# linnil1/KIR_graph

Measured on AMD Instinct MI355X. Metric: typed 150 bp PE reads/s (pileup+EM) per GPU; achieved HBM GB/s vs roofline, higher is better.
Workload: dtype f64

## Files before the change

include/graphkir_hip.h:

```cpp
#ifndef GRAPHKIR_HIP_H
#define GRAPHKIR_HIP_H

#include <stddef.h>
#include <stdint.h>

#ifdef __cplusplus
extern "C" {
#endif

#define GK_ABI_VERSION 1

#define GK_OK 0
#define GK_ERR_NO_DEVICE (-1)
#define GK_ERR_HIP (-2)
#define GK_ERR_ARG (-3)
#define GK_ERR_ASSERT (-4)
#define GK_ERR_CAPACITY (-5)

#define GK_MAX_CIG 14
#define GK_MAX_MM 16
#define GK_MAX_INS 6
#define GK_MAX_EVENTS 22
#define GK_CIG_M 0
#define GK_CIG_I 1
// ... 47 lines not shown
typedef struct gk_tab gk_tab;
typedef struct gk_lut gk_lut;
typedef uint64_t gk_dptr;

int gk_abi_version(void);
const char* gk_last_error(void);
int gk_device_count(int* n);
int gk_ctx_create(int device, gk_ctx** out);
int gk_ctx_create_priority(int device, int urgent, gk_ctx** out);
int gk_ctx_destroy(gk_ctx* ctx);
int gk_sync(gk_ctx* ctx);
int gk_device_memory(gk_ctx* ctx, int64_t* free_bytes, int64_t* total_bytes, int64_t* pool_cached_bytes);
int gk_malloc(gk_ctx* ctx, size_t bytes, gk_dptr* out);
int gk_free(gk_ctx* ctx, gk_dptr p);
int gk_memset(gk_ctx* ctx, gk_dptr p, int value, size_t bytes);
int gk_h2d(gk_ctx* ctx, gk_dptr dst, const void* src, size_t bytes);
int gk_d2h(gk_ctx* ctx, void* dst, gk_dptr src, size_t bytes);
int gk_d2d(gk_ctx* ctx, gk_dptr dst, gk_dptr src, size_t bytes);
int gk_timer_start(gk_ctx* ctx);
int gk_timer_stop_ms(gk_ctx* ctx, float* ms);
int gk_prof_enable(gk_ctx* ctx, int on);
int gk_prof_kernel_count(void);
const char* gk_prof_kernel_name(int id);
int gk_prof_collect(gk_ctx* ctx, int64_t* launches, double* total_ms);

int gk_index_create(gk_ctx* ctx, const uint64_t* key, int32_t n_var, const int32_t* gene_vbeg,
                    int32_t n_gene, gk_index** out);
int gk_index_destroy(gk_index* idx);

typedef struct gk_tab_info {
  int64_t n_pairs;
  int64_t n_valid;
  int64_t n_ids;
  int32_t n_novel;
  int32_t err_flags;
  gk_dptr d_pair_src;
  gk_dptr d_off;
  gk_dptr d_ids;
  gk_dptr d_pair_gene;
  gk_dptr d_pair_nh;
  gk_dptr d_novel_key;
} gk_tab_info;
int gk_tabulate(gk_ctx* ctx, gk_index* idx, gk_dptr d_mates, int64_t n_pairs, gk_tab** out);
int gk_tabulate_corrected(gk_ctx* ctx, gk_index* idx, gk_dptr d_mates, int64_t n_pairs, gk_dptr d_corr,
                          gk_dptr d_gene_pos0, gk_tab** out);
int gk_tabulate_spilled(gk_ctx* ctx, gk_index* idx, gk_dptr d_mates, int64_t n_pairs, gk_dptr d_corr,
                        gk_dptr d_gene_pos0, const gk_mate_wide* wide, const int64_t* spill_pair, int64_t n_spill,
                        gk_tab** out);
#define GK_COMPACT_STAGE_WORDS 4352
int gk_tabulate_compact(gk_ctx* ctx, gk_index* idx, gk_dptr d_compact, int64_t n_pairs, gk_dptr d_corr,
                        gk_dptr d_gene_pos0, const gk_mate_wide* wide, const int64_t* spill_pair, int64_t n_spill,
                        gk_tab** out);
int gk_tab_from_csr(gk_ctx* ctx, int32_t n_var_total, int64_t n_valid, const uint32_t* off, const uint32_t* ids,
                    const uint8_t* pair_gene, const uint8_t* pair_nh, gk_tab** out);
int gk_tab_get_info(gk_tab* tab, gk_tab_info* info);
int gk_tab_destroy(gk_tab* tab);

int gk_select_gene(gk_ctx* ctx, gk_tab* tab, int gene, int multiple, gk_dptr d_rows_out, int64_t* n_out);
int gk_select_nonempty(gk_ctx* ctx, gk_tab* tab, gk_dptr d_rows, int64_t n_rows, gk_dptr d_vflag,
                       gk_dptr d_rows_out, int64_t* n_out);

int gk_variant_count(gk_ctx* ctx, gk_tab* tab, gk_dptr d_rows, int64_t n_rows, gk_dptr d_vflag,
                     gk_dptr d_cnt);
int gk_variant_count_range(gk_ctx* ctx, gk_tab* tab, gk_dptr d_rows, int64_t n_rows, gk_dptr d_vflag,
                           gk_dptr d_cnt, int32_t vbeg, int32_t vend);
int gk_variant_correct(gk_ctx* ctx, gk_tab* tab, gk_dptr d_cnt, gk_dptr d_vflag);
int gk_variant_surviving(gk_ctx* ctx, gk_tab* tab, gk_dptr d_cnt, gk_dptr d_vflag, int64_t max_out,
                         int32_t* ord_out, uint32_t* pos_out, uint32_t* neg_out, int64_t* n_out);

int gk_variant_surviving_gene(gk_ctx* ctx, gk_tab* tab, gk_dptr d_cnt, gk_dptr d_vflag, int32_t gene, int32_t vbeg,
                              int32_t vend, int64_t max_out, int32_t* ord_out, uint32_t* pos_out, uint32_t* neg_out,
                              int64_t* n_out);
int gk_sample_prepare(gk_ctx* ctx, gk_tab* tab, int32_t multiple, gk_dptr d_vflag, gk_dptr d_cnt, gk_dptr d_rows,
                      int64_t* gene_off_out);
int gk_sample_prepare_all(gk_ctx* ctx, gk_tab* tab, int32_t multiple, gk_dptr d_vflag, gk_dptr d_cnt, gk_dptr d_rows,
                          int64_t* gene_off_out, int64_t max_out, int32_t* ord_out, uint32_t* pos_out, uint32_t* neg_out,
                          int64_t* n_out, uint64_t* novel_key_out);
int gk_sample_prepare_exon(gk_ctx* ctx, gk_tab* tab, int32_t multiple, gk_dptr d_vflag, gk_dptr d_cnt, gk_dptr d_rows,
                           int64_t* gene_off_out, int64_t max_out, int32_t* ord_out, uint32_t* pos_out, uint32_t* neg_out,
                           int64_t* n_out);
int gk_sample_prepare_exon_from(gk_ctx* ctx, gk_tab* tab, int32_t multiple, gk_dptr d_vflag, gk_dptr d_cnt, gk_dptr d_rows,
                                int64_t* gene_off_out, int64_t max_out, int32_t* ord_out, uint32_t* pos_out,
                                uint32_t* neg_out, int64_t* n_out, gk_dptr d_cnt_full);

int gk_compat(gk_ctx* ctx, gk_tab* tab, gk_dptr d_rows, int64_t n_rows, gk_dptr d_vflag,
              int32_t vbeg, int32_t vend, gk_dptr d_mask, int32_t words, int32_t n_allele, int32_t keep_empty,
              gk_dptr d_probs, gk_dptr d_miss, gk_dptr d_nvar);

int gk_novel_assign(gk_ctx* ctx, gk_dptr d_probs, int64_t n_rows, int32_t n_cols, const uint32_t* col_entries,
                    int32_t n_entries, gk_dptr d_code, uint16_t* code_out, uint32_t* count_out, int32_t* first_out);
int gk_novel_confusion(gk_ctx* ctx, gk_tab* tab, gk_dptr d_rows, int64_t n_rows, gk_dptr d_code, gk_dptr d_vflag,
                       int32_t vbeg, int32_t vend, gk_dptr d_carry, const int32_t* entry_col, const int32_t* entry_slot,
                       int32_t n_entries, int32_t n_slots, uint64_t* totals_out, int64_t max_out, int32_t* slot_out,
                       int32_t* ord_out, uint32_t* count_out, uint64_t* key_out, int64_t* n_out);

int gk_lut_create(gk_ctx* ctx, int32_t log2_capacity, gk_lut** out);
int gk_lut_destroy(gk_lut* lut);
int gk_lut_collect(gk_lut* lut, gk_dptr d_vals, int64_t n);
int gk_lut_pending(gk_lut* lut, int32_t* n_total, int32_t* n_known);
int gk_lut_export(gk_lut* lut, int32_t first, int32_t count, double* keys_out);
int gk_lut_define(gk_lut* lut, int32_t first, int32_t count, const double* log_vals);
int gk_lut_apply(gk_lut* lut, gk_dptr d_in, gk_dptr d_out, int64_t n);
typedef int (*gk_log10_fn)(const double* values, int64_t n, double* out);
int gk_lut_resolve(gk_lut* lut, gk_log10_fn log10_fn, int32_t* n_new, int32_t* n_known, int32_t* n_undefined);
int gk_lut_resolve_stored(gk_lut* lut, gk_log10_fn log10_fn, int32_t* n_new, int32_t* n_known, int32_t* n_undefined);
int gk_lut_known(gk_lut* lut, int32_t* n_known);
int gk_compat_log(gk_ctx* ctx, gk_tab* tab, gk_dptr d_rows, int64_t n_rows, gk_dptr d_vflag,
                  int32_t vbeg, int32_t vend, gk_dptr d_mask, int32_t words, int32_t n_allele, int32_t keep_empty,
                  gk_lut* lut, gk_dptr d_log);

int gk_maxsum(gk_ctx* ctx, gk_dptr d_L, int64_t n_rows, int64_t ld, const int32_t* ids, int32_t n_sets,
              int32_t c_prev, const int32_t* cols, int32_t n_cols, double* out);
int gk_fraction(gk_ctx* ctx, gk_dptr d_L, int64_t n_rows, int64_t ld, const int32_t* ids,
                int32_t n_sets, int32_t c, double* frac_out);
int gk_setmax(gk_ctx* ctx, gk_dptr d_L, int64_t n_rows, int64_t ld, const int32_t* ids, int32_t n_sets,
              int32_t c, gk_dptr d_P);

int gk_compat_log_miss(gk_ctx* ctx, gk_tab* tab, gk_dptr d_rows, int64_t n_rows, gk_dptr d_vflag,
                       int32_t vbeg, int32_t vend, gk_dptr d_mask, int32_t words, int32_t n_allele,
                       int32_t keep_empty, gk_lut* lut, gk_dptr d_log, gk_dptr d_miss8, int64_t ldm, gk_dptr d_flags);
int gk_miss_colsum(gk_ctx* ctx, gk_dptr d_miss8, int64_t ldm, int32_t n_cols, gk_dptr d_msum);
int gk_compat_log_miss_cols(gk_ctx* ctx, gk_tab* tab, gk_dptr d_rows, int64_t n_rows, gk_dptr d_vflag,
                            int32_t vbeg, int32_t vend, gk_dptr d_mask, int32_t words, int32_t n_allele,
                            int32_t keep_empty, gk_lut* lut, const int32_t* table_cols, int32_t n_table_cols,
                            gk_dptr d_log, gk_dptr d_miss8, int64_t ldm, gk_dptr d_flags);
int gk_compat_log_miss_narrow(gk_ctx* ctx, gk_tab* tab, gk_dptr d_rows, int64_t n_rows, gk_dptr d_vflag,
                              int32_t vbeg, int32_t vend, gk_dptr d_mask, int32_t words, int32_t n_allele,
                              int32_t keep_empty, gk_lut* lut, const int32_t* table_cols, int32_t n_table_cols,
                              gk_dptr d_log, gk_dptr d_miss8, int64_t ldm, gk_dptr d_flags, gk_dptr d_msum);
int gk_compat_patch(gk_ctx* ctx, gk_lut* lut, gk_dptr d_log, int64_t n_rows, int32_t n_allele, gk_dptr d_miss8,
                    int64_t ldm, gk_dptr d_flags);
int gk_compat_index(gk_ctx* ctx, gk_tab* tab, gk_dptr d_rows, int64_t n_rows, gk_dptr d_vflag, int32_t vbeg,
                    int32_t vend, gk_dptr d_mask, int32_t words, int32_t n_allele, int32_t keep_empty, gk_lut* lut,
                    gk_dptr d_lidx, gk_dptr d_miss8, int64_t ldm, gk_dptr d_flags);
int gk_expand_index(gk_ctx* ctx, gk_lut* lut, gk_dptr d_lidx, int64_t ldi, int64_t n_rows, int32_t n_allele, gk_dptr d_L,
                    int64_t ld);
int gk_bound_step(gk_ctx* ctx, gk_dptr d_miss8, int64_t ldm, int64_t n_rows, gk_dptr d_msum, const int32_t* ids,
                  int32_t n_sets, int32_t c_prev, const int32_t* cols, int32_t n_cols, const uint8_t* first,
                  int32_t top_n, int32_t cap, uint32_t* hdr_out, int32_t* idx_out, uint32_t* m_out);
int gk_setsum(gk_ctx* ctx, gk_dptr d_L, int64_t n_rows, int64_t ld, const int32_t* ids, int32_t n_sets, int32_t c,
              double* value_out, double* frac_out);

typedef int (*gk_argsort_fn)(const double* values, int64_t n, int64_t* order_out);
typedef struct gk_search gk_search;
int gk_search_run(gk_ctx* ctx, gk_dptr d_L, int64_t n_rows, int64_t ld, int32_t n_allele, gk_dptr d_miss8,
                  int64_t ldm, gk_dptr d_msum, const int32_t* cols, int32_t n_cols, int32_t n_steps, int32_t top_n,
                  gk_argsort_fn argsort, const double* colsum_in, gk_search** out);
typedef struct gk_gene_job {
  gk_dptr d_rows;
  int64_t n_rows;
  gk_dptr d_mask;
  gk_dptr d_L;
  gk_dptr d_miss8;
  int64_t ldm;
  gk_dptr d_msum;
  gk_dptr d_flags;
  gk_dptr d_lidx;
  int32_t vbeg, vend;
  int32_t words, n_allele;
  int32_t n_steps, top_n;
  int32_t bound_ok, passes;
  int32_t indexed, patches;
  int32_t table_of, n_step_cols;
  const int32_t* step_cols;
  const int32_t* step_cols_off;
  const int32_t* table_cols;
  int32_t n_table_cols;
} gk_gene_job;
int gk_sample_search(gk_ctx* ctx, gk_ctx** more_ctx, int32_t n_more, gk_tab* tab, gk_dptr d_vflag, gk_lut* lut,
                     gk_gene_job* jobs, int32_t n_jobs, gk_argsort_fn argsort, gk_log10_fn log10_fn, gk_search** out);
int gk_search_steps(gk_search* s, int32_t* n_steps);
int gk_search_info(gk_search* s, int32_t step, int32_t* n, int64_t* rows, int32_t* bounded);
int gk_search_copy(gk_search* s, int32_t step, double* value, double* sum_indv, int32_t* ids, double* frac);
int gk_search_export(gk_search* const* s, int32_t n, int64_t* totals, int64_t* meta, double* value, double* sum_indv,
                     double* frac, int32_t* ids);
int gk_search_colsum(gk_search* s, double* out);
int gk_search_log(gk_search* s, int64_t* out, int64_t capacity, int64_t* n_out);
int gk_search_destroy(gk_search* s);
int gk_site_verdict(const int64_t* pos, const int64_t* code, const uint8_t* negative, const int64_t* count, int64_t n,
                    int32_t cn, int32_t* homozygous);
int gk_site_verdict_tallies(const uint64_t* keys, int64_t n_keys, const int64_t* label_of_insert, int64_t n_insert,
                            const int32_t* ordinal, const uint32_t* positive, const uint32_t* negative, int64_t n,
                            int32_t cn, int32_t* homozygous);
int gk_site_verdict_genes(const uint64_t* keys, int64_t n_keys, const int64_t* label_of_insert, int64_t n_insert,
                          const int32_t* ordinal, const uint32_t* positive, const uint32_t* negative,
                          const int64_t* bounds, int32_t n_groups, const int32_t* cn, int32_t* homozygous);

int gk_em_sets(gk_ctx* ctx, gk_tab* tab, gk_dptr d_rows, int64_t n_rows, int32_t vbeg, int32_t vend,
               gk_dptr d_mask, int32_t words, gk_dptr d_sets_out );
int gk_em_distinct(gk_ctx* ctx, gk_dptr d_sets, int64_t n_rows, int32_t words, int32_t max_out,
                   uint32_t* sets_out, uint32_t* count_out, int32_t* n_out);
int gk_em_run(gk_ctx* ctx, const uint32_t* sets, const double* weight, int32_t n_sets, int32_t words,
              int32_t n_allele, int32_t iter_max, double diff_threshold, double* prob_out,
              int32_t* iters_out);
typedef struct gk_em_job {
  gk_dptr d_rows;
  int64_t n_rows;
  gk_dptr d_mask;
  int32_t vbeg, vend;
  int32_t words, n_allele;
  int32_t n_distinct, iterations;
} gk_em_job;
int gk_sample_em(gk_ctx* ctx, gk_tab* tab, gk_em_job* jobs, int32_t n_jobs, int32_t iter_max, double diff_threshold,
                 double* prob_out, int64_t* count_out);

typedef struct gk_boot_job {
  const uint32_t* sets;
  const uint32_t* count;
  int32_t n_sets;
  int32_t words;
  int32_t n_allele;
  uint32_t stream;
// ... 100 lines not shown
```

kir_graph_amd/_lib.py:

```python
from __future__ import annotations

import ctypes as C
import threading
import os
from pathlib import Path

import numpy as np

LIB_NAME = "libgraphkir_hip.so"
_lib = None


class GkError(RuntimeError):
    """Error reported by the native library."""


class GkNoDevice(GkError):
    """No HIP device: the typing path cannot run (there is no CPU fallback)."""


_MM = np.dtype([("ref_off", "<u2"), ("base", "u1"), ("rsv", "u1")])
MATE_DTYPE = np.dtype([
    ("pos0", "<u4"), ("flag", "<u2"), ("ref", "u1"), ("nh", "u1"),
    ("nm", "u1"), ("n_cig", "u1"), ("n_mm", "u1"), ("n_ins", "u1"),
# ... 95 lines not shown
                                     C.POINTER(C.c_int64)]),
    "gk_variant_count": (C.c_int, [C.c_void_p, C.c_void_p, C.c_uint64, C.c_int64, C.c_uint64, C.c_uint64]),
    "gk_variant_count_range": (C.c_int, [C.c_void_p, C.c_void_p, C.c_uint64, C.c_int64, C.c_uint64, C.c_uint64,
                                         C.c_int32, C.c_int32]),
    "gk_variant_surviving": (C.c_int, [C.c_void_p, C.c_void_p, C.c_uint64, C.c_uint64, C.c_int64, C.c_void_p,
                                       C.c_void_p, C.c_void_p, C.POINTER(C.c_int64)]),
    "gk_variant_surviving_gene": (C.c_int, [C.c_void_p, C.c_void_p, C.c_uint64, C.c_uint64, C.c_int32, C.c_int32, C.c_int32,
                                            C.c_int64, C.c_void_p, C.c_void_p, C.c_void_p, C.POINTER(C.c_int64)]),
    "gk_sample_prepare": (C.c_int, [C.c_void_p, C.c_void_p, C.c_int32, C.c_uint64, C.c_uint64, C.c_uint64, C.c_void_p]),
    "gk_sample_prepare_all": (C.c_int, [C.c_void_p, C.c_void_p, C.c_int32, C.c_uint64, C.c_uint64, C.c_uint64, C.c_void_p,
                                       C.c_int64, C.c_void_p, C.c_void_p, C.c_void_p, C.POINTER(C.c_int64), C.c_void_p]),
    "gk_variant_correct": (C.c_int, [C.c_void_p, C.c_void_p, C.c_uint64, C.c_uint64]),
    "gk_compat": (C.c_int, [C.c_void_p, C.c_void_p, C.c_uint64, C.c_int64, C.c_uint64, C.c_int32, C.c_int32,
                            C.c_uint64, C.c_int32, C.c_int32, C.c_int32, C.c_uint64, C.c_uint64, C.c_uint64]),
    "gk_lut_create": (C.c_int, [C.c_void_p, C.c_int32, C.POINTER(C.c_void_p)]),
    "gk_lut_destroy": (C.c_int, [C.c_void_p]),
    "gk_lut_collect": (C.c_int, [C.c_void_p, C.c_uint64, C.c_int64]),
    "gk_lut_pending": (C.c_int, [C.c_void_p, C.POINTER(C.c_int32), C.POINTER(C.c_int32)]),
    "gk_lut_export": (C.c_int, [C.c_void_p, C.c_int32, C.c_int32, C.c_void_p]),
    "gk_lut_define": (C.c_int, [C.c_void_p, C.c_int32, C.c_int32, C.c_void_p]),
    "gk_lut_apply": (C.c_int, [C.c_void_p, C.c_uint64, C.c_uint64, C.c_int64]),
    "gk_bam_open": (C.c_int, [C.c_char_p, C.c_int32, C.POINTER(C.c_void_p)]),
    "gk_bam_close": (C.c_int, [C.c_void_p]),
    "gk_bam_info": (C.c_int, [C.c_void_p, C.POINTER(C.c_int64), C.POINTER(C.c_int64), C.POINTER(C.c_int32)]),
    "gk_bam_header": (C.c_int, [C.c_void_p, C.c_char_p, C.c_int64]),
    "gk_bam_pileup": (C.c_int, [C.c_void_p, C.c_void_p, C.c_int32, C.c_void_p]),
    "gk_bam_pileup_sites": (C.c_int, [C.c_char_p, C.c_void_p, C.c_int64, C.c_void_p, C.c_void_p, C.c_int64, C.c_void_p,
                                      C.c_void_p]),
    "gk_sam_name_keys": (C.c_int, [C.c_char_p, C.c_int64, C.c_void_p, C.c_int64, C.c_void_p]),
    "gk_bam_write_lines_tagged": (C.c_int, [C.c_char_p, C.c_char_p, C.c_int64, C.c_char_p, C.c_int64, C.c_char_p,
                                            C.c_int64, C.c_void_p, C.c_void_p, C.c_int64, C.c_void_p, C.c_int32,
                                            C.c_int32]),
    "gk_novel_assign": (C.c_int, [C.c_void_p, C.c_uint64, C.c_int64, C.c_int32, C.c_void_p, C.c_int32, C.c_uint64,
                                  C.c_void_p, C.c_void_p, C.c_void_p]),
    "gk_novel_confusion": (C.c_int, [C.c_void_p, C.c_void_p, C.c_uint64, C.c_int64, C.c_uint64, C.c_uint64, C.c_int32,
                                     C.c_int32, C.c_uint64, C.c_void_p, C.c_void_p, C.c_int32, C.c_int32, C.c_void_p,
                                     C.c_int64, C.c_void_p, C.c_void_p, C.c_void_p, C.c_void_p, C.POINTER(C.c_int64)]),
    "gk_bam_write": (C.c_int, [C.c_char_p, C.c_char_p, C.c_int64, C.c_int32]),
    "gk_bam_write_lines": (C.c_int, [C.c_char_p, C.c_char_p, C.c_int64, C.c_char_p, C.c_int64, C.c_void_p, C.c_int64,
                                     C.c_int32]),
    "gk_json_write_reads": (C.c_int, [C.c_char_p, C.c_char_p, C.c_int64, C.c_void_p, C.c_int64, C.c_void_p, C.c_int64,
                                      C.c_void_p, C.c_void_p, C.c_void_p, C.c_int64, C.c_void_p, C.c_int32,
                                      C.c_void_p, C.c_void_p]),
    "gk_bam_pack": (C.c_int, [C.c_void_p, C.c_void_p]),
    "gk_bam_next": (C.c_int, [C.c_void_p, C.c_void_p, C.c_int64, C.POINTER(C.c_int64)]),
    "gk_compat_log": (C.c_int, [C.c_void_p, C.c_void_p, C.c_uint64, C.c_int64, C.c_uint64, C.c_int32, C.c_int32,
                                C.c_uint64, C.c_int32, C.c_int32, C.c_int32, C.c_void_p, C.c_uint64]),
    "gk_maxsum": (C.c_int, [C.c_void_p, C.c_uint64, C.c_int64, C.c_int64, C.c_void_p, C.c_int32, C.c_int32,
                            C.c_void_p, C.c_int32, C.c_void_p]),
    "gk_fraction": (C.c_int, [C.c_void_p, C.c_uint64, C.c_int64, C.c_int64, C.c_void_p, C.c_int32, C.c_int32,
                              C.c_void_p]),
    "gk_setmax": (C.c_int, [C.c_void_p, C.c_uint64, C.c_int64, C.c_int64, C.c_void_p, C.c_int32, C.c_int32,
                            C.c_uint64]),
    "gk_packer_create": (C.c_int, [C.c_void_p, C.c_int32, C.c_void_p, C.c_int32, C.POINTER(C.c_void_p)]),
    "gk_packer_destroy": (C.c_int, [C.c_void_p]),
    "gk_packer_feed": (C.c_int, [C.c_void_p, C.c_char_p, C.c_size_t, C.c_int32]),
    "gk_packer_counts": (C.c_int, [C.c_void_p, C.POINTER(C.c_int64), C.POINTER(C.c_int64), C.POINTER(C.c_int64),
                                   C.POINTER(C.c_int64), C.POINTER(C.c_int64)]),
    "gk_packer_error": (C.c_int, [C.c_void_p, C.POINTER(C.c_int32), C.POINTER(C.c_int64)]),
    "gk_packer_records": (C.c_int, [C.c_void_p, C.c_void_p, C.c_void_p]),
    "gk_packer_set_output": (C.c_int, [C.c_void_p, C.c_void_p, C.c_int64]),
    "gk_packer_spilled": (C.c_int, [C.c_void_p, C.POINTER(C.c_int64)]),
    "gk_packer_spill_records": (C.c_int, [C.c_void_p, C.c_void_p, C.c_void_p]),
    "gk_packer_string": (C.c_char_p, [C.c_void_p, C.c_int64]),
    "gk_depth": (C.c_int, [C.c_void_p, C.c_void_p, C.c_uint64, C.c_int32, C.c_void_p, C.c_int32, C.c_void_p]),
    "gk_depth_compact": (C.c_int, [C.c_void_p, C.c_void_p, C.c_uint64, C.c_int32, C.c_void_p, C.c_int32, C.c_void_p]),
    "gk_depth_weighted": (C.c_int, [C.c_void_p, C.c_void_p, C.c_uint64, C.c_uint64, C.c_int32, C.c_void_p, C.c_int32, C.c_uint64,
                                    C.c_int64, C.c_int32, C.c_void_p, C.c_void_p, C.c_void_p, C.c_void_p, C.c_void_p]),
    "gk_depth_write_tsv": (C.c_int, [C.c_char_p, C.c_void_p, C.c_void_p, C.c_int32, C.c_void_p]),
    "gk_cn_fit": (C.c_int, [C.c_void_p, C.c_void_p, C.c_void_p, C.c_int32, C.c_void_p, C.c_int32, C.c_void_p,
                            C.c_int32, C.c_int32, C.c_double, C.c_void_p]),
    "gk_cn_assign": (C.c_int, [C.c_void_p, C.c_void_p, C.c_int32, C.c_double, C.c_void_p, C.c_int32, C.c_int32,
                               C.c_double, C.c_void_p]),
    "gk_em_sets": (C.c_int, [C.c_void_p, C.c_void_p, C.c_uint64, C.c_int64, C.c_int32, C.c_int32, C.c_uint64,
                             C.c_int32, C.c_uint64]),
    "gk_em_distinct": (C.c_int, [C.c_void_p, C.c_uint64, C.c_int64, C.c_int32, C.c_int32, C.c_void_p, C.c_void_p,
                                 C.POINTER(C.c_int32)]),
    "gk_compat_log_miss_cols": (C.c_int, [C.c_void_p, C.c_void_p, C.c_uint64, C.c_int64, C.c_uint64, C.c_int32, C.c_int32,
                                          C.c_uint64, C.c_int32, C.c_int32, C.c_int32, C.c_void_p, C.c_void_p, C.c_int32,
                                          C.c_uint64, C.c_uint64, C.c_int64, C.c_uint64]),
    "gk_compat_log_miss_narrow": (C.c_int, [C.c_void_p, C.c_void_p, C.c_uint64, C.c_int64, C.c_uint64, C.c_int32, C.c_int32,
                                            C.c_uint64, C.c_int32, C.c_int32, C.c_int32, C.c_void_p, C.c_void_p, C.c_int32,
                                            C.c_uint64, C.c_uint64, C.c_int64, C.c_uint64, C.c_uint64]),
    "gk_compat_log_miss": (C.c_int, [C.c_void_p, C.c_void_p, C.c_uint64, C.c_int64, C.c_uint64, C.c_int32, C.c_int32,
                                     C.c_uint64, C.c_int32, C.c_int32, C.c_int32, C.c_void_p, C.c_uint64, C.c_uint64,
                                     C.c_int64, C.c_uint64]),
    "gk_miss_colsum": (C.c_int, [C.c_void_p, C.c_uint64, C.c_int64, C.c_int32, C.c_uint64]),
    "gk_compat_index": (C.c_int, [C.c_void_p, C.c_void_p, C.c_uint64, C.c_int64, C.c_uint64, C.c_int32, C.c_int32,
                                  C.c_uint64, C.c_int32, C.c_int32, C.c_int32, C.c_void_p, C.c_uint64, C.c_uint64,
                                  C.c_int64, C.c_uint64]),
    "gk_expand_index": (C.c_int, [C.c_void_p, C.c_void_p, C.c_uint64, C.c_int64, C.c_int64, C.c_int32, C.c_uint64,
                                  C.c_int64]),
    "gk_bound_step": (C.c_int, [C.c_void_p, C.c_uint64, C.c_int64, C.c_int64, C.c_uint64, C.c_void_p, C.c_int32,
                                C.c_int32, C.c_void_p, C.c_int32, C.c_void_p, C.c_int32, C.c_int32, C.c_void_p,
                                C.c_void_p, C.c_void_p]),
    "gk_setsum": (C.c_int, [C.c_void_p, C.c_uint64, C.c_int64, C.c_int64, C.c_void_p, C.c_int32, C.c_int32,
                            C.c_void_p, C.c_void_p]),
    "gk_search_run": (C.c_int, [C.c_void_p, C.c_uint64, C.c_int64, C.c_int64, C.c_int32, C.c_uint64, C.c_int64,
                                C.c_uint64, C.c_void_p, C.c_int32, C.c_int32, C.c_int32, C.c_void_p, C.c_void_p,
                                C.POINTER(C.c_void_p)]),
    "gk_sample_search": (C.c_int, [C.c_void_p, C.c_void_p, C.c_int32, C.c_void_p, C.c_uint64, C.c_void_p, C.c_void_p,
                                   C.c_int32, C.c_void_p, C.c_void_p, C.c_void_p]),
    "gk_lut_resolve": (C.c_int, [C.c_void_p, C.c_void_p, C.POINTER(C.c_int32), C.POINTER(C.c_int32),
                                 C.POINTER(C.c_int32)]),
    "gk_sample_prepare_exon": (C.c_int, [C.c_void_p, C.c_void_p, C.c_int32, C.c_uint64, C.c_uint64, C.c_uint64, C.c_void_p,
                                         C.c_int64, C.c_void_p, C.c_void_p, C.c_void_p, C.POINTER(C.c_int64)]),
    "gk_sample_prepare_exon_from": (C.c_int, [C.c_void_p, C.c_void_p, C.c_int32, C.c_uint64, C.c_uint64, C.c_uint64, C.c_void_p,
                                              C.c_int64, C.c_void_p, C.c_void_p, C.c_void_p, C.POINTER(C.c_int64), C.c_uint64]),
    "gk_sample_em": (C.c_int, [C.c_void_p, C.c_void_p, C.c_void_p, C.c_int32, C.c_int32, C.c_double, C.c_void_p, C.c_void_p]),
    "gk_mates_compact": (C.c_int, [C.c_void_p, C.c_uint64, C.c_int64, C.POINTER(C.c_uint64), C.POINTER(C.c_int64)]),
    "gk_mates_expand": (C.c_int, [C.c_void_p, C.c_uint64, C.c_int64, C.c_uint64]),
    "gk_mates_compact_size": (C.c_int, [C.c_void_p, C.c_int64, C.c_int32, C.POINTER(C.c_int64)]),
    "gk_mates_compact_host": (C.c_int, [C.c_void_p, C.c_int64, C.c_int32, C.c_void_p, C.c_int64]),
    "gk_compat_patch": (C.c_int, [C.c_void_p, C.c_void_p, C.c_uint64, C.c_int64, C.c_int32, C.c_uint64, C.c_int64, C.c_uint64]),
    "gk_lut_resolve_stored": (C.c_int, [C.c_void_p, C.c_void_p, C.POINTER(C.c_int32), C.POINTER(C.c_int32),
                                        C.POINTER(C.c_int32)]),
    "gk_lut_known": (C.c_int, [C.c_void_p, C.POINTER(C.c_int32)]),
    "gk_search_steps": (C.c_int, [C.c_void_p, C.POINTER(C.c_int32)]),
    "gk_search_info": (C.c_int, [C.c_void_p, C.c_int32, C.POINTER(C.c_int32), C.POINTER(C.c_int64),
                                 C.POINTER(C.c_int32)]),
    "gk_search_copy": (C.c_int, [C.c_void_p, C.c_int32, C.c_void_p, C.c_void_p, C.c_void_p, C.c_void_p]),
    "gk_search_export": (C.c_int, [C.c_void_p, C.c_int32, C.c_void_p, C.c_void_p, C.c_void_p, C.c_void_p, C.c_void_p, C.c_void_p]),
    "gk_search_colsum": (C.c_int, [C.c_void_p, C.c_void_p]),
    "gk_search_log": (C.c_int, [C.c_void_p, C.c_void_p, C.c_int64, C.POINTER(C.c_int64)]),
    "gk_search_destroy": (C.c_int, [C.c_void_p]),
    "gk_site_verdict_tallies": (C.c_int, [C.c_void_p, C.c_int64, C.c_void_p, C.c_int64, C.c_void_p, C.c_void_p, C.c_void_p,
                                         C.c_int64, C.c_int32, C.POINTER(C.c_int32)]),
    "gk_site_verdict_genes": (C.c_int, [C.c_void_p, C.c_int64, C.c_void_p, C.c_int64, C.c_void_p, C.c_void_p, C.c_void_p,
                                       C.c_void_p, C.c_int32, C.c_void_p, C.c_void_p]),
    "gk_site_verdict": (C.c_int, [C.c_void_p, C.c_void_p, C.c_void_p, C.c_void_p, C.c_int64, C.c_int32,
                                  C.POINTER(C.c_int32)]),
    "gk_comm_unique_id": (C.c_int, [C.c_void_p, C.c_size_t]),
    "gk_comm_create": (C.c_int, [C.c_void_p, C.c_void_p, C.c_size_t, C.c_int32, C.c_int32, C.POINTER(C.c_void_p)]),
    "gk_comm_destroy": (C.c_int, [C.c_void_p]),
    "gk_allgather_f64": (C.c_int, [C.c_void_p, C.c_void_p, C.c_void_p, C.c_int64]),
    "gk_allreduce_max_f64": (C.c_int, [C.c_void_p, C.c_void_p, C.c_int64]),
    "gk_comm_barrier": (C.c_int, [C.c_void_p]),
    "gk_host_alloc": (C.c_int, [C.c_size_t, C.POINTER(C.c_void_p)]),
    "gk_host_free": (C.c_int, [C.c_void_p]),
    "gk_h2d_async": (C.c_int, [C.c_void_p, C.c_uint64, C.c_void_p, C.c_size_t]),
    "gk_em_run": (C.c_int, [C.c_void_p, C.c_void_p, C.c_void_p, C.c_int32, C.c_int32, C.c_int32, C.c_int32,
                            C.c_double, C.c_void_p, C.POINTER(C.c_int32)]),
    "gk_em_bootstrap": (C.c_int, [C.c_void_p, C.c_void_p, C.c_int32, C.c_int32, C.c_uint64, C.c_int32, C.c_double,
                                  C.c_void_p, C.c_void_p, C.c_void_p]),
    "gk_boot_row_counts": (C.c_int, [C.c_void_p, C.c_int64, C.c_int32, C.c_int32, C.c_uint64, C.c_uint32, C.c_uint64,
                                     C.c_int64]),
    "gk_weighted_sums": (C.c_int, [C.c_void_p, C.c_uint64, C.c_int64, C.c_int64, C.c_int32, C.c_uint64, C.c_int64, C.c_int32,
                                   C.c_void_p]),
    "gk_call_fit": (C.c_int, [C.c_void_p, C.c_uint64, C.c_int64, C.c_int64, C.c_int32, C.c_void_p, C.c_int32, C.c_void_p,
                              C.c_void_p, C.c_void_p, C.c_uint64]),
    "gk_call_fit_extra": (C.c_int, [C.c_void_p, C.c_uint64, C.c_int64, C.c_int64, C.c_int32, C.c_uint64, C.c_void_p]),
    "gk_call_coverage": (C.c_int, [C.c_void_p, C.c_void_p, C.c_uint64, C.c_uint64, C.c_uint64, C.c_int64, C.c_uint64, C.c_int64,
                                   C.c_int32, C.c_void_p, C.c_int32, C.c_int32, C.c_int64, C.c_void_p]),
}

EXPORTED = sorted(_SIGS)

ARGSORT_FN = C.CFUNCTYPE(C.c_int, C.POINTER(C.c_double), C.c_int64, C.POINTER(C.c_int64))


def _numpy_argsort(values, n, order_out):
    try:
        v = np.ctypeslib.as_array(values, shape=(n,))
        np.ctypeslib.as_array(order_out, shape=(n,))[:] = np.argsort(v)
        return 0
    except Exception:
        return 1


NUMPY_ARGSORT = ARGSORT_FN(_numpy_argsort)

LOG10_FN = C.CFUNCTYPE(C.c_int, C.POINTER(C.c_double), C.c_int64, C.POINTER(C.c_double))


def _numpy_log10(values, n, out):
    try:
        v = np.ctypeslib.as_array(values, shape=(n,))
        with np.errstate(divide="ignore"):
            np.ctypeslib.as_array(out, shape=(n,))[:] = np.log10(v)
        return 0
    except Exception:
        return 1


NUMPY_LOG10 = LOG10_FN(_numpy_log10)


def lib():
    global _lib
    if _lib is None:
        path = libPath()
# ... 224 lines not shown
```

kir_graph_amd/csrc/gk_hostsearch.cpp:

```cpp
#include <algorithm>
#include <cmath>
#include <memory>
#include <numeric>
#include <string>
#include <unordered_map>
#include <unordered_set>
#include <chrono>
#include <sys/syscall.h>
#include <unistd.h>

#include "gk_calls.h"
#include "gk_lut.h"

namespace {

struct Step {
  int n = 0;
  int bounded = 0;
  std::vector<double> value, sum_indv, frac;
  std::vector<int32_t> ids;
  int64_t rows() const { return (int64_t)value.size(); }
};

inline double sum_small(const double* a, int n) {
// ... 94 lines not shown
  }
}

void contenders(const Head& h, int top_n, std::vector<int64_t>& contend) {
  const int64_t n = (int64_t)h.value.size();
  contend.clear();
  if (n <= top_n) {
    contend.resize((size_t)n);
    std::iota(contend.begin(), contend.end(), 0);
    return;
  }
  std::vector<int64_t> order((size_t)n);
  std::iota(order.begin(), order.end(), 0);
  std::stable_sort(order.begin(), order.end(), [&](int64_t a, int64_t b) {
    const double ka = -h.value[a], kb = -h.value[b];
    if (ka != kb) return ka < kb;
    return h.key2[a] < h.key2[b];
  });
  const int64_t b = order[top_n - 1];
  const double b1 = -h.value[b], b2 = h.key2[b];
  for (int64_t i = 0; i < n; ++i) {
    const double k1 = -h.value[i];
    if (k1 < b1 || (k1 == b1 && h.key2[i] <= b2)) contend.push_back(i);
  }
}

double unevenness(const double* f, int c) {
  const double mean = sum_small(f, c) / (double)c;
  double d[8];
  for (int j = 0; j < c; ++j) d[j] = std::fabs(f[j] - mean);
  return sum_small(d, c);
}

}

struct gk_search {
  int n_allele = 0;
  std::vector<int32_t> table_cols;
  int n_full = 0;
  std::vector<double> colsum;
  std::vector<Step> steps;
  std::vector<int64_t> log;
  int64_t distinct(const int32_t* ids, size_t n) const {
    std::vector<char> seen((size_t)n_allele, 0);
    int64_t d = 0;
    for (size_t i = 0; i < n; ++i)
      if (!seen[ids[i]]) { seen[ids[i]] = 1; ++d; }
    return d;
  }
  void note(int64_t kind, int64_t a, int64_t b, int64_t c, int64_t d, int64_t e, int64_t f) {
    const int64_t row[7] = {kind, a, b, c, d, e, f};
    log.insert(log.end(), row, row + 7);
  }
  void to_alleles(const int32_t* cols, int n_cols, int n_alleles) {
    for (Step& st : steps)
      for (int32_t& id : st.ids) id = cols[id];
    table_cols.assign(cols, cols + n_cols);
    n_full = n_alleles;
  }
};

extern "C" {

int gk_maxsum(gk_ctx* ctx, gk_dptr d_L, int64_t n_rows, int64_t ld, const int32_t* ids, int32_t n_sets, int32_t c_prev,
              const int32_t* cols, int32_t n_cols, double* out);
int gk_fraction(gk_ctx* ctx, gk_dptr d_L, int64_t n_rows, int64_t ld, const int32_t* ids, int32_t n_sets, int32_t c,
                double* frac_out);
int gk_compat_log_miss(gk_ctx* ctx, gk_tab* tab, gk_dptr d_rows, int64_t n_rows, gk_dptr d_vflag, int32_t vbeg,
                       int32_t vend, gk_dptr d_mask, int32_t words, int32_t n_allele, int32_t keep_empty, gk_lut* lut,
                       gk_dptr d_log, gk_dptr d_miss8, int64_t ldm, gk_dptr d_flags);
int gk_compat_log(gk_ctx* ctx, gk_tab* tab, gk_dptr d_rows, int64_t n_rows, gk_dptr d_vflag, int32_t vbeg,
                  int32_t vend, gk_dptr d_mask, int32_t words, int32_t n_allele, int32_t keep_empty, gk_lut* lut,
                  gk_dptr d_log);
__attribute__((weak)) int gk_compat_log_miss_cols(gk_ctx* ctx, gk_tab* tab, gk_dptr d_rows, int64_t n_rows, gk_dptr d_vflag,
                                                  int32_t vbeg, int32_t vend, gk_dptr d_mask, int32_t words, int32_t n_allele,
                                                  int32_t keep_empty, gk_lut* lut, const int32_t* table_cols,
                                                  int32_t n_table_cols, gk_dptr d_log, gk_dptr d_miss8, int64_t ldm,
                                                  gk_dptr d_flags);
__attribute__((weak)) int gk_compat_log_miss_narrow(gk_ctx* ctx, gk_tab* tab, gk_dptr d_rows, int64_t n_rows, gk_dptr d_vflag,
                                                    int32_t vbeg, int32_t vend, gk_dptr d_mask, int32_t words, int32_t n_allele,
                                                    int32_t keep_empty, gk_lut* lut, const int32_t* table_cols,
                                                    int32_t n_table_cols, gk_dptr d_log, gk_dptr d_miss8, int64_t ldm,
                                                    gk_dptr d_flags, gk_dptr d_msum);
int gk_miss_colsum(gk_ctx* ctx, gk_dptr d_miss8, int64_t ldm, int32_t n_cols, gk_dptr d_msum);
int gk_compat_patch(gk_ctx* ctx, gk_lut* lut, gk_dptr d_log, int64_t n_rows, int32_t n_allele, gk_dptr d_miss8, int64_t ldm,
                    gk_dptr d_flags);
int gk_compat_index(gk_ctx* ctx, gk_tab* tab, gk_dptr d_rows, int64_t n_rows, gk_dptr d_vflag, int32_t vbeg, int32_t vend,
                    gk_dptr d_mask, int32_t words, int32_t n_allele, int32_t keep_empty, gk_lut* lut, gk_dptr d_lidx,
                    gk_dptr d_miss8, int64_t ldm, gk_dptr d_flags);

}

namespace {

struct GeneSearch {
  gk_ctx* ctx = nullptr;
  GkTable table;
  gk_dptr d_L = 0;
  void* expanded = nullptr;
  gk_dptr d_miss8 = 0, d_msum = 0;
  int64_t n_rows = 0, ld = 0, ldm = 0;
  int n_allele = 0, n_steps = 0, T = 0, A = 0;
  std::vector<int32_t> cols;
  std::vector<std::vector<int32_t>> step_cols;
  gk_argsort_fn argsort = nullptr;
  bool bound = false, unique_cols = true;
  std::unique_ptr<gk_search> S;
  std::vector<uint8_t> first;
  int64_t N = 0;
  GkBoundCall bcall;
  GkSumCall scall;
  Head sel;
  Step st;
  bool bound_in_flight = false, sums_in_flight = false, step_done = false;

  int init(gk_ctx* c, const GkTable& tbl, gk_dptr L, int64_t rows, int64_t ld_, int32_t n_allele_, gk_dptr miss8, int64_t ldm_,
           gk_dptr msum, const int32_t* cols_, int32_t n_cols, int32_t n_steps_, int32_t top_n, gk_argsort_fn fn) {
    GK_REQUIRE(c && tbl.d && (L || tbl.indexed()) && cols_ && fn, "null pointer");
    table = tbl;
    GK_REQUIRE(rows > 0 && ld_ >= rows && n_allele_ > 0 && n_cols > 0 && n_steps_ >= 0 && n_steps_ <= 8 && top_n >= 1,
               "bad search arguments");
    for (int a = 0; a < n_cols; ++a) GK_REQUIRE(cols_[a] >= 0 && cols_[a] < n_allele_, "candidate allele out of range");
    ctx = c; d_L = L; n_rows = rows; ld = ld_; n_allele = n_allele_; d_miss8 = miss8; ldm = ldm_; d_msum = msum;
    cols.assign(cols_, cols_ + n_cols);
    n_steps = n_steps_; T = top_n; A = n_cols; argsort = fn;
    bound = d_miss8 != 0 && d_msum != 0;
    S.reset(new gk_search());
    S->n_allele = n_allele;
    S->colsum.resize((size_t)n_allele);
    std::vector<char> seen((size_t)n_allele, 0);
    for (int a = 0; a < A && unique_cols; ++a) { if (seen[cols[a]]) unique_cols = false; seen[cols[a]] = 1; }
    return GK_OK;
  }

  int use_step(int s) {
    if (step_cols.empty()) return GK_OK;
    const std::vector<int32_t>& c = step_cols[std::min<size_t>((size_t)s, step_cols.size() - 1)];
    GK_REQUIRE(!c.empty(), "a search step without candidate alleles");
    cols = c;
    A = (int)cols.size();
    unique_cols = true;
    std::vector<char> seen((size_t)n_allele, 0);
    for (int a = 0; a < A; ++a) {
      GK_REQUIRE(cols[a] >= 0 && cols[a] < n_allele, "candidate allele out of range");
      if (seen[cols[a]]) unique_cols = false;
      seen[cols[a]] = 1;
    }
    return GK_OK;
  }

  int colsum_enqueue() {
    std::vector<int32_t> every((size_t)n_allele);
    std::iota(every.begin(), every.end(), 0);
    int rc = gk_colsum_enqueue(ctx, table, n_rows, every.data(), n_allele, scall);
    if (rc) return rc;
    S->note(0, n_rows, 1, 0, n_allele, 0, 0);
    return GK_OK;
  }
  void colsum_collect() { gk_colsum_collect(ctx, scall, S->colsum.data()); }

  int first_step() {
    { const int r = use_step(0); if (r) return r; }
    const double* colsum = S->colsum.data();
    std::vector<double> score((size_t)A);
    for (int a = 0; a < A; ++a) score[a] = colsum[cols[a]];
    std::vector<int64_t> order((size_t)A);
// ... 460 lines not shown
    lap(false); rc = wait_all(); lap(true);
    if (rc) return fail(rc);
  }
  for (int i : live) {
    gs[i]->colsum_collect();
    rc = gs[i]->first_step();
    if (rc) return fail(rc);
  }
  for (;;) {
    std::vector<int> todo;
    for (int i : live) if (gs[i]->more()) todo.push_back(i);
    if (todo.empty()) break;
    for (int i : todo) { rc = gs[i]->step_begin(); if (rc) return fail(rc); }
    lap(false); rc = wait_all(); lap(true);
    if (rc) return fail(rc);
    for (int i : todo) { rc = gs[i]->after_bound(); if (rc) return fail(rc); }
    lap(false); rc = wait_all(); lap(true);
    if (rc) return fail(rc);
    for (int i : todo) { rc = gs[i]->after_sums(); if (rc) return fail(rc); }
    for (int i : todo) {
      if (!gs[i]->step_done) { rc = gs[i]->exact_step(); if (rc) return fail(rc); }
      gs[i]->step_end();
    }
  }
  for (int i : live) {
    gs[i]->finish();
    out[i] = gs[i]->S.release();
  }
  for (int i = 0; i < n_jobs; ++i) gk_pool_free(ctx_of[i], own_L[i]);
  lap(false);
  return GK_OK;
}

int sample_search_pipelined(gk_ctx* ctx, gk_tab* tab, gk_dptr d_vflag, gk_lut* lut, gk_gene_job* jobs, int32_t n_jobs,
                            const std::vector<int>& live, gk_argsort_fn argsort, gk_log10_fn log10_fn, gk_search** out) {
  SearchClock clock("pipelined", (int)live.size());
  std::vector<uint32_t> flags((size_t)n_jobs, 0);
  std::vector<std::unique_ptr<GeneSearch>> gs((size_t)n_jobs);
  enum { kTable, kBound, kSums, kOneSet };
  struct Item { int gene, stage; uint64_t mark; };
  std::deque<Item> queue;
  struct OneSetBatch { GkSumCall call; std::vector<int> deps; int k = 0; std::vector<int32_t> ids; };
  std::vector<std::unique_ptr<OneSetBatch>> batches;
  auto fail = [&](int code) {
    gk_fetch_cancel(ctx);
    for (auto& g : gs) if (g) g->abandon();
    for (auto& b : batches) if (b) gk_release(ctx, b->call.temps);
    return code;
  };
  auto push = [&](int gene, int stage) {
    uint64_t m = 0;
    const int r = set_mark(ctx, &m);
    if (r == GK_OK) queue.push_back({gene, stage, m});
    return r;
  };
  std::vector<uint32_t> sticky((size_t)n_jobs, 0);
  auto n_cols_of = [&](int i) { return jobs[i].n_table_cols > 0 ? jobs[i].n_table_cols : jobs[i].n_allele; };
  auto col_of = [&](int owner, int32_t a, int32_t* col) -> int {
    const gk_gene_job& o = jobs[owner];
    if (a < 0 || a >= o.n_allele) { gk_set_error("candidate allele out of range"); return GK_ERR_ARG; }
    if (o.n_table_cols <= 0) { *col = a; return GK_OK; }
    const int32_t* const end = o.table_cols + o.n_table_cols;
    const int32_t* const at = std::lower_bound(o.table_cols, end, a);
    if (at == end || *at != a) {
      gk_set_error("candidate allele %d is not among the columns of its table", (int)a);
      return GK_ERR_ARG;
    }
    *col = (int32_t)(at - o.table_cols);
    return GK_OK;
  };
  auto write_table = [&](int i, bool patch) -> int {
    gk_gene_job& j = jobs[i];
    const int nc = n_cols_of(i);
    int rc;
    bool summed = false;
    if (patch) {
      j.patches++;
      sticky[i] |= flags[i] & 1u;
      rc = gk_compat_patch(ctx, lut, j.d_L, j.n_rows, nc, j.d_miss8, j.ldm, j.d_flags);
    } else {
      j.passes++;
      sticky[i] = 0;
      static const bool wide_compat = gk_test_hook("wide_compat");
      if (j.n_table_cols > 0 && j.n_table_cols <= 8 && gk_compat_log_miss_narrow && !wide_compat) {
        rc = gk_compat_log_miss_narrow(ctx, tab, j.d_rows, j.n_rows, d_vflag, j.vbeg, j.vend, j.d_mask, j.words, j.n_allele, 0,
                                       lut, j.table_cols, j.n_table_cols, j.d_L, j.d_miss8, j.ldm, j.d_flags, j.d_msum);
        summed = true;
      } else if (j.n_table_cols > 0)
        rc = gk_compat_log_miss_cols(ctx, tab, j.d_rows, j.n_rows, d_vflag, j.vbeg, j.vend, j.d_mask, j.words, j.n_allele, 0,
                                     lut, j.table_cols, j.n_table_cols, j.d_L, j.d_miss8, j.ldm, j.d_flags);
      else
        rc = gk_compat_log_miss(ctx, tab, j.d_rows, j.n_rows, d_vflag, j.vbeg, j.vend, j.d_mask, j.words, j.n_allele, 0, lut,
                                j.d_L, j.d_miss8, j.ldm, j.d_flags);
    }
    if (rc == GK_OK && !summed) rc = gk_miss_colsum(ctx, j.d_miss8, j.ldm, nc, j.d_msum);
    if (rc == GK_OK && gk_fetch_queue(ctx, &flags[i], gk_ptr<void>(j.d_flags), sizeof(uint32_t)) != hipSuccess) rc = GK_ERR_HIP;
    if (rc) return rc;
    std::vector<int32_t> cols((size_t)nc);
    std::iota(cols.begin(), cols.end(), 0);
    if (gs[i]) gs[i]->abandon();
    gs[i].reset(new GeneSearch());
    rc = gs[i]->init(ctx, GkTable{j.d_L, j.n_rows, nullptr}, j.d_L, j.n_rows, j.n_rows, nc, j.d_miss8, j.ldm, j.d_msum,
                     cols.data(), nc, j.n_steps, j.top_n, argsort);
    if (rc == GK_OK) rc = gs[i]->colsum_enqueue();
    if (rc == GK_OK) rc = push(i, kTable);
    return rc;
  };
  std::vector<std::vector<int>> dependents((size_t)n_jobs);
  for (int i : live)
    if (jobs[i].table_of >= 0) dependents[(size_t)jobs[i].table_of].push_back(i);
  int rc = GK_OK;
  for (int i : live) {
    if (jobs[i].table_of >= 0) continue;
    rc = write_table(i, false);
    if (rc) return fail(rc);
  }

  auto advance = [&](int i, bool at_step_start) -> int {
    GeneSearch& g = *gs[i];
    for (;;) {
      if (at_step_start) {
        if (!g.more()) return GK_OK;
        const int r = g.step_begin();
        if (r) return r;
        if (g.bound_in_flight) return push(i, kBound);
      }
      if (!g.step_done) {
        const int r = g.exact_step();
        if (r) return r;
      }
      g.step_end();
      at_step_start = true;
    }
  };
  while (!queue.empty()) {
    const Item it = queue.front();
    queue.pop_front();
    clock.lap(false);
    rc = wait_mark(ctx, it.mark);
    clock.lap(true);
    if (rc) return fail(rc);
    const int at = it.stage == kOneSet ? batches[(size_t)it.gene]->deps[0] : it.gene;
    gk_gene_job& j = jobs[at];
    GeneSearch& g = *gs[at];
    switch (it.stage) {
      case kTable: {
        if (flags[it.gene] & 4u) {
          if (j.passes + j.patches >= 64) {
            gk_set_error("log10 value table did not settle");
            rc = GK_ERR_ASSERT;
            break;
          }
          rc = (j.passes + j.patches < 4 ? gk_lut_resolve_stored : gk_lut_resolve)(lut, log10_fn, nullptr, nullptr, nullptr);
          if (rc == GK_OK) rc = write_table(it.gene, (flags[it.gene] & 8u) == 0);
          break;
        }
        j.bound_ok = ((flags[it.gene] | sticky[it.gene]) & 1u) == 0 ? 1 : 0;
        if (!j.bound_ok) g.bound = false;
        g.colsum_collect();
        if (j.n_steps > 0) {
          rc = g.first_step();
          if (rc == GK_OK) rc = advance(it.gene, true);
        }
        const int nc = n_cols_of(it.gene);
        std::vector<int> one_set;
        for (int d : dependents[(size_t)it.gene]) {
          if (rc) break;
          gk_gene_job& jd = jobs[d];
          jd.bound_ok = j.bound_ok;
// ... 331 lines not shown
```

kir_graph_amd/csrc/gk_typing.hip:

```cpp
#include <algorithm>

#include "gk_common.h"
#include "gk_lut.h"

namespace {

constexpr int kThreads = 256;
inline unsigned nblk(int64_t n, int t = kThreads) { return (unsigned)((n + t - 1) / t); }

template <bool kScatter>
__global__ __launch_bounds__(kThreads) void part_pass(const uint8_t* gene, const uint8_t* nh, int64_t n, int multiple,
                                                      int n_bins, int64_t n_tiles, uint32_t* hist, int32_t* out) {
  const int64_t i = (int64_t)blockIdx.x * kThreads + threadIdx.x;
  const int lane = threadIdx.x & 63;
  const int64_t tile = i >> 6;
  int bin = -1;
  if (i < n && (multiple || nh[i] == 1)) {
    bin = gene[i];
    if (bin >= n_bins) bin = -1;
  }
  uint64_t todo = __ballot(bin >= 0);
  while (todo) {
    const int leader = __ffsll((unsigned long long)todo) - 1;
    const int b = __shfl(bin, leader, 64);
// ... 6 lines not shown
    todo &= ~same;
  }
}

__global__ void part_offsets(const uint32_t* hist, const uint32_t* total, int n_bins, int64_t n_tiles, uint32_t* goff) {
  const int b = blockIdx.x * blockDim.x + threadIdx.x;
  if (b < n_bins) goff[b] = hist[(int64_t)b * n_tiles];
  if (b == n_bins) goff[b] = *total;
}

__global__ __launch_bounds__(kThreads) void count_ids(const int32_t* __restrict__ rows, int64_t n_rows,
                                                      const uint32_t* __restrict__ off,
                                                      const uint32_t* __restrict__ ids,
                                                      const uint8_t* __restrict__ vflag, uint32_t* cnt_pos,
                                                      uint32_t* cnt_neg, int vbeg, int n_local) {
  extern __shared__ uint32_t hist[];
  for (int i = threadIdx.x; i < 2 * n_local; i += kThreads) hist[i] = 0;
  __syncthreads();
  constexpr int kGroup = 16;
  const int lane = threadIdx.x & (kGroup - 1);
  const int64_t group = ((int64_t)blockIdx.x * kThreads + threadIdx.x) / kGroup;
  const int64_t n_groups = ((int64_t)gridDim.x * kThreads) / kGroup;
  for (int64_t i = group; i < n_rows; i += n_groups) {
    const int64_t row = rows[i];
    const uint32_t b = off[4 * row], mid = off[4 * row + 2], e = off[4 * row + 4];
    for (uint32_t k = b + lane; k < e; k += kGroup) {
      const uint32_t v = ids[k];
      const bool positive = k < mid;
      if (vflag[v] & (positive ? 1 : 2)) continue;
      const uint32_t l = v - (uint32_t)vbeg;
      if (l < (uint32_t)n_local) atomicAdd(&hist[(positive ? 0 : n_local) + l], 1u);
      else atomicAdd(positive ? &cnt_pos[v] : &cnt_neg[v], 1u);
    }
  }
  __syncthreads();
  for (int i = threadIdx.x; i < 2 * n_local; i += kThreads) {
    const uint32_t c = hist[i];
    if (c) atomicAdd(i < n_local ? &cnt_pos[vbeg + i] : &cnt_neg[vbeg + i - n_local], c);
  }
}

__global__ __launch_bounds__(kThreads) void apply_correction(const uint32_t* cnt_pos, const uint32_t* cnt_neg,
                                                             int64_t n, uint8_t* vflag) {
  const int64_t v = (int64_t)blockIdx.x * kThreads + threadIdx.x;
  if (v >= n) return;
  const uint64_t p = cnt_pos[v], q = cnt_neg[v];
  if (p + q == 0) return;
  uint8_t f = vflag[v];
  if (p + q < 3) {
    f |= 3;
  } else {
    if (5 * p < p + q) f |= 1;
    if (5 * q < p + q) f |= 2;
  }
  vflag[v] = f;
}

__global__ __launch_bounds__(kThreads) void mask_tallies(const uint32_t* __restrict__ full_pos,
                                                         const uint32_t* __restrict__ full_neg,
                                                         const uint8_t* __restrict__ vflag, int64_t n,
                                                         uint32_t* __restrict__ cnt_pos, uint32_t* __restrict__ cnt_neg) {
  const int64_t v = (int64_t)blockIdx.x * kThreads + threadIdx.x;
  if (v >= n) return;
  const uint8_t f = vflag[v];
  cnt_pos[v] = (f & 1) ? 0u : full_pos[v];
  cnt_neg[v] = (f & 2) ? 0u : full_neg[v];
}

__global__ __launch_bounds__(kThreads) void flag_nonempty(const int32_t* rows, int64_t n_rows, const uint32_t* off,
                                                          const uint32_t* ids, const uint8_t* vflag, uint32_t* flag,
                                                          uint32_t* zero, int n_zero) {
  const int64_t i = (int64_t)blockIdx.x * kThreads + threadIdx.x;
  if (zero && i < n_zero) zero[i] = 0;
  if (i >= n_rows) return;
  const int64_t row = rows[i];
  const uint32_t b = off[4 * row], mid = off[4 * row + 2], e = off[4 * row + 4];
  uint32_t alive = 0;
  for (uint32_t k = b; k < e && !alive; ++k) alive = !(vflag[ids[k]] & (k < mid ? 1 : 2));
  flag[i] = alive;
}

__global__ __launch_bounds__(kThreads) void flag_pairs(int64_t n_pairs, const uint32_t* __restrict__ off,
                                                       const uint32_t* __restrict__ ids, const uint8_t* __restrict__ vflag,
                                                       const uint8_t* __restrict__ maybe, uint8_t* __restrict__ alive) {
  const int64_t t = (int64_t)blockIdx.x * kThreads + threadIdx.x;
  const int64_t p = t >> 2;
  const uint32_t l = (uint32_t)t & 3u;
  uint32_t b = 0, mid = 0, e = 0;
  if (p < n_pairs && maybe[p]) { b = off[4 * p]; mid = off[4 * p + 2]; e = off[4 * p + 4]; }
  const int shift = (threadIdx.x & 63) & ~3;
  bool any = false;
  for (uint32_t k0 = b; k0 < e && !any; k0 += 4) {
    const uint32_t k = k0 + l;
    const bool mine = k < e && !(vflag[ids[k]] & (k < mid ? 1 : 2));
    any = ((__ballot(mine) >> shift) & 0xFull) != 0ull;
  }
  if (p < n_pairs && l == 0) alive[p] = any ? 1 : 0;
}

__global__ __launch_bounds__(kThreads) void gather_pair_flags(const int32_t* __restrict__ rows, int64_t n_rows,
                                                              const uint8_t* __restrict__ alive, uint32_t* __restrict__ flag,
                                                              uint32_t* zero, int n_zero) {
  const int64_t i = (int64_t)blockIdx.x * kThreads + threadIdx.x;
  if (zero && i < n_zero) zero[i] = 0;
  if (i < n_rows) flag[i] = alive[rows[i]];
}

__global__ __launch_bounds__(kThreads) void count_ids_genes(const int32_t* __restrict__ rows,
                                                            const int32_t* __restrict__ wg_gene,
                                                            const int64_t* __restrict__ wg_row0,
                                                            const int64_t* __restrict__ wg_row1,
                                                            const int32_t* __restrict__ gene_vbeg, int max_local,
                                                            const uint32_t* __restrict__ off,
                                                            const uint32_t* __restrict__ ids,
                                                            const uint8_t* __restrict__ vflag, uint32_t* cnt_pos,
                                                            uint32_t* cnt_neg, uint8_t* __restrict__ maybe) {
  extern __shared__ uint32_t hist[];
  const int g = wg_gene[blockIdx.x];
  const int vbeg = gene_vbeg[g];
  const int n_local = min(gene_vbeg[g + 1] - vbeg, max_local);
  for (int i = threadIdx.x; i < 2 * n_local; i += kThreads) hist[i] = 0;
  __syncthreads();
  constexpr int kGroup = 16, kDeep = 4;
  const int lane = threadIdx.x & (kGroup - 1);
  uint32_t* const spare = hist + 2 * max_local + threadIdx.x;
  const int64_t r0 = wg_row0[blockIdx.x], r1 = wg_row1[blockIdx.x];
  constexpr int64_t kStep = kThreads / kGroup;
  int64_t i = r0 + threadIdx.x / kGroup;
  auto row_at = [&](int64_t j) { return rows[j < r1 ? j : r1 - 1]; };
  int32_t row = row_at(i), row1 = row_at(i + kStep);
  uint32_t b = off[4 * (int64_t)row], mid = off[4 * (int64_t)row + 2], e = off[4 * (int64_t)row + 4];
  if (i >= r1) b = mid = e = 0u;
  auto tally = [&](uint32_t k0, const uint32_t (&v)[kDeep], const uint8_t (&f)[kDeep]) {
    bool counted = false;
#pragma unroll
    for (int j = 0; j < kDeep; ++j) {
      const uint32_t k = k0 + kGroup * j;
      const bool positive = k < mid;
      const bool counts = k < e && !(f[j] & (positive ? 1 : 2));
      const uint32_t l = v[j] - (uint32_t)vbeg;
      const bool local = l < (uint32_t)n_local;
      atomicAdd((counts && local) ? &hist[(positive ? 0 : n_local) + l] : spare, (counts && local) ? 1u : 0u);
      if (counts && !local) atomicAdd(positive ? &cnt_pos[v[j]] : &cnt_neg[v[j]], 1u);
      counted = counted || counts;
    }
    return counted;
  };
  auto ids_of = [&](uint32_t k0, uint32_t (&v)[kDeep]) {
    const uint32_t last = e ? e - 1u : 0u;
#pragma unroll
    for (int j = 0; j < kDeep; ++j) v[j] = ids[k0 + kGroup * j < e ? k0 + kGroup * j : last];
  };
  for (; i < r1; i += kStep) {
    uint32_t v[kDeep];
    uint8_t f[kDeep];
    ids_of(b + lane, v);
    const int64_t next = row1;
    const uint32_t nb = off[4 * next], nmid = off[4 * next + 2], ne = off[4 * next + 4];
    row1 = row_at(i + 2 * kStep);
#pragma unroll
    for (int j = 0; j < kDeep; ++j) f[j] = vflag[v[j]];
    bool counted = tally(b + lane, v, f);
    for (uint32_t k0 = b + kGroup * kDeep + lane; k0 < e; k0 += kGroup * kDeep) {
      ids_of(k0, v);
#pragma unroll
      for (int j = 0; j < kDeep; ++j) f[j] = vflag[v[j]];
      counted = tally(k0, v, f) || counted;
    }
    if (maybe) {
      const bool any = ((__ballot(counted) >> ((threadIdx.x & 63) & ~(kGroup - 1))) & 0xFFFFull) != 0ull;
      if (lane == 0) maybe[row] = any ? 1 : 0;
    }
    row = (int32_t)next;
    const bool more = i + kStep < r1;
    b = more ? nb : 0u; mid = more ? nmid : 0u; e = more ? ne : 0u;
  }
  __syncthreads();
  for (int i2 = threadIdx.x; i2 < 2 * n_local; i2 += kThreads) {
    const uint32_t c = hist[i2];
    if (c) atomicAdd(i2 < n_local ? &cnt_pos[vbeg + i2] : &cnt_neg[vbeg + i2 - n_local], c);
  }
}

constexpr int kFlagSlices = 16;
__global__ __launch_bounds__(kThreads) void count_flags_per_gene(const uint32_t* __restrict__ flag,
                                                                 const int64_t* __restrict__ gene_off,
                                                                 uint32_t* __restrict__ kept) {
  const int g = blockIdx.x;
  const int64_t g0 = gene_off[g], g1 = gene_off[g + 1];
  const int64_t per = (g1 - g0 + gridDim.y - 1) / gridDim.y;
  const int64_t a = g0 + per * blockIdx.y, b = min(g1, a + per);
  uint32_t c = 0;
  for (int64_t i = a + threadIdx.x; i < b; i += kThreads) c += flag[i] != 0;
  __shared__ uint32_t part[kThreads];
  part[threadIdx.x] = c;
  __syncthreads();
  for (int s2 = kThreads / 2; s2 > 0; s2 >>= 1) {
    if (threadIdx.x < s2) part[threadIdx.x] += part[threadIdx.x + s2];
    __syncthreads();
  }
  if (threadIdx.x == 0 && part[0]) atomicAdd(&kept[g], part[0]);
}

constexpr int kMaxSlots = 4;
constexpr int kCompatWaves = 8;
constexpr int kCompatThreads = 64 * kCompatWaves;
constexpr int kTileRows = 16;
constexpr int kTileLd = kTileRows + 1;

__global__ __launch_bounds__(kThreads) void transpose_mask(const uint32_t* mask, int n_span, int words, uint32_t* out,
                                                           uint32_t* zero_word) {
  if (zero_word && blockIdx.x == 0 && threadIdx.x == 0) *zero_word = 0;
  const int64_t i = (int64_t)blockIdx.x * kThreads + threadIdx.x;
  if (i >= (int64_t)n_span * words) return;
  const int w = (int)(i / n_span), v = (int)(i % n_span);
  out[i] = mask[(int64_t)v * words + w];
}

__global__ __launch_bounds__(kThreads) void transpose_gather_mask(const uint32_t* __restrict__ mask, int n_span, int words,
                                                                  const int32_t* __restrict__ cols, int n_cols,
                                                                  int words_out, uint32_t* __restrict__ out,
                                                                  uint32_t* zero_word) {
  if (zero_word && blockIdx.x == 0 && threadIdx.x == 0) *zero_word = 0;
  const int64_t i = (int64_t)blockIdx.x * kThreads + threadIdx.x;
  if (i >= (int64_t)n_span * words_out) return;
  const int w = (int)(i / n_span), v = (int)(i % n_span);
  const uint32_t* const row = mask + (int64_t)v * words;
  const int n_bits = min(32, n_cols - 32 * w);
  uint32_t x = 0;
  for (int b = 0; b < n_bits; ++b) {
    const int a = cols[32 * w + b];
    x |= ((row[a >> 5] >> (a & 31)) & 1u) << b;
  }
  out[i] = x;
}

constexpr uint16_t kNoIndex = 0xFFFFu;

template <bool kLog, int kSlots, bool kMiss, bool kIdx>
__global__ __launch_bounds__(kCompatThreads) void compat_kernel(const int32_t* rows, int64_t n_rows, const uint32_t* off,
                                                                const uint32_t* ids, const uint8_t* vflag, int vbeg, int vend,
                                                                const uint32_t* mask_t, int words, int n_allele, int a_base,
                                                                double* probs, uint8_t* miss_out, uint16_t* nvar_out,
                                                                LutView lut, double empty_p, uint8_t* miss8, int64_t ldm,
                                                                uint32_t* bound_flags, uint16_t* lidx) {
  const int n_span = vend - vbeg;
  constexpr int kPassAlleles = 64 * kSlots;
  constexpr int kPassWords = 2 * kSlots;
  __shared__ double tile[kPassAlleles * kTileLd];
  __shared__ uint32_t wave_rows[kCompatWaves][65 * kPassWords];
  constexpr int32_t kHi999 = 0x3FEFF7CE, kLo999 = (int32_t)0xD916872B, kHi001 = 0x3F50624D, kLo001 = (int32_t)0xD2F1A9FC;
  const int tid = threadIdx.x, lane = tid & 63;
  const int wid = __builtin_amdgcn_readfirstlane(tid >> 6);
  const int w_base = a_base >> 5;

  int a[kSlots];
  bool live[kSlots];
#pragma unroll
  for (int s = 0; s < kSlots; ++s) {
    a[s] = a_base + lane + 64 * s;
    live[s] = a[s] < n_allele;
  }
  const int n_pass = min(kPassAlleles, n_allele - a_base);
  const int64_t n_tiles = (n_rows + kTileRows - 1) / kTileRows;
  const int64_t n_groups = (n_tiles + 7) / 8;
  const int xcd = blockIdx.x & 7;
  const int64_t my_groups = n_groups > xcd ? (n_groups - xcd + 7) / 8 : 0;
  const int64_t wg_per_xcd = gridDim.x >> 3;
  for (int64_t u = blockIdx.x >> 3; u < 8 * my_groups; u += wg_per_xcd) {
    const int64_t tile_i = 8 * (xcd + 8 * (u >> 3)) + (u & 7);
    if (tile_i >= n_tiles) continue;
    const int64_t row0 = tile_i * kTileRows;
    constexpr int kRowsPerWave = kTileRows / kCompatWaves;
    uint32_t row_b[kRowsPerWave], row_mid[kRowsPerWave], row_e[kRowsPerWave];
#pragma unroll
    for (int q = 0; q < kRowsPerWave; ++q) {
      const int64_t i = row0 + wid * kRowsPerWave + q;
      const int64_t row = rows[i < n_rows ? i : n_rows - 1];
      row_b[q] = off[4 * row]; row_mid[q] = off[4 * row + 2]; row_e[q] = off[4 * row + 4];
    }
    uint32_t first_id[kRowsPerWave];
#pragma unroll
    for (int q = 0; q < kRowsPerWave; ++q) {
      const uint32_t k = row_b[q] + (uint32_t)lane;
      first_id[q] = ids[k < row_e[q] ? k : (row_e[q] ? row_e[q] - 1u : 0u)];
    }
#pragma unroll
    for (int q = 0; q < kRowsPerWave; ++q) {
      const int rt = wid * kRowsPerWave + q;
      const int64_t i = row0 + rt;
      if (i >= n_rows) break;
      const uint32_t b = __builtin_amdgcn_readfirstlane(row_b[q]);
      const uint32_t mid = __builtin_amdgcn_readfirstlane(row_mid[q]);
      const uint32_t e = __builtin_amdgcn_readfirstlane(row_e[q]);
      double p[kSlots];
      uint32_t miss[kSlots];
      uint32_t nvar = 0;
#pragma unroll
      for (int s = 0; s < kSlots; ++s) { p[s] = 1.0; miss[s] = 0; }
      const uint32_t* const my_words = &wave_rows[wid][lane >> 5];
      const int my_bit = lane & 31;
      for (uint32_t base = b; base < e; base += 64) {
        const uint32_t k = base + lane;
        const bool in = k < e;
        const uint32_t v = base == b ? first_id[q] : ids[in ? k : e - 1u];
        const uint32_t local = v - (uint32_t)vbeg;
        const bool indexed = local < (uint32_t)n_span;
        const uint32_t at = indexed ? local : 0u;
        const uint8_t dropped = vflag[v];
        const uint32_t flip = k >= mid ? 0xFFFFFFFFu : 0u;
        uint32_t mrow[kPassWords];
#pragma unroll
        for (int w = 0; w < kPassWords; ++w) {
          const bool has = w + 1 < kPassWords || w_base + w < words;
          const uint32_t* const col = mask_t + (int64_t)(has ? w_base + w : 0) * n_span;
          const uint32_t x = col[at];
          mrow[w] = ((indexed && has) ? x : 0u) ^ flip;
        }
        const bool my_keep = in && !(dropped & (k < mid ? 1 : 2));
        const uint64_t kept = __ballot(my_keep);
        const int n_kept = __builtin_popcountll(kept);
        nvar += (uint32_t)n_kept;
        {
          const uint32_t place = __builtin_amdgcn_mbcnt_hi((uint32_t)(kept >> 32), __builtin_amdgcn_mbcnt_lo((uint32_t)kept, 0u));
          uint32_t* const dst = &wave_rows[wid][(my_keep ? place : 64u) * kPassWords];
#pragma unroll
          for (int w = 0; w < kPassWords; ++w) dst[w] = mrow[w];
        }
        __builtin_amdgcn_wave_barrier();
        auto apply = [&](const uint32_t (&w)[kSlots]) {
#pragma unroll
          for (int s = 0; s < kSlots; ++s) {
            const int32_t m = __builtin_amdgcn_sbfe((int32_t)w[s], my_bit, 1);
// ... 67 lines not shown
        x = (uint32_t)__builtin_amdgcn_update_dpp(0, (int)x, 0xF9, 0xF, 0xF, true);
        packed |= x << 24;
        const uint32_t i1 = (uint32_t)__builtin_amdgcn_update_dpp(0, (int)id16, 0xF9, 0xF, 0xF, true);
        const uint32_t i2 = (uint32_t)__builtin_amdgcn_update_dpp(0, (int)i1, 0xF9, 0xF, 0xF, true);
        const uint32_t i3 = (uint32_t)__builtin_amdgcn_update_dpp(0, (int)i2, 0xF9, 0xF, 0xF, true);
        if ((r & 3) == 0) {
          const int64_t at = (int64_t)(a_base + al) * ldm + row0 + r;
          *reinterpret_cast<uint32_t*>(miss8 + at) = packed;
          *reinterpret_cast<uint2*>(lidx + at) = make_uint2(id16 | (i1 << 16), i2 | (i3 << 16));
        }
      }
    } else
    if (probs) {
      const int n_r = (int)min<int64_t>(kTileRows, n_rows - row0);
      if (kLog) {
        uint64_t key0 = kLutEmptyKey, key1 = kLutEmptyKey;
        double val0 = 0.0, val1 = 0.0;
        uint32_t raise = 0;
        constexpr int kRowThreads = kCompatThreads / kTileRows;
        const int per_thread = (n_pass + kRowThreads - 1) / kRowThreads;
        const int r = tid % kTileRows, al0 = (tid / kTileRows) * per_thread;
        for (int al = al0; al < min(al0 + per_thread, n_pass); ++al) {
          if (r >= n_r) break;
          double* const cell = &tile[al * kTileLd + r];
          const uint64_t key = (uint64_t)__double_as_longlong(*cell);
          if (key != key0) {
            double val;
            if (key == key1) {
              val = val1;
            } else {
              bool found;
              val = gk_lut_lookup(lut, key, &found);
              if (!found) {
                gk_lut_insert(lut, key);
                if (bound_flags) {
                  const bool marks = (int64_t)key > 0;
                  raise |= marks ? 4u : 12u;
                  if (marks) val = __longlong_as_double((long long)key);
                }
              }
            }
            key1 = key0; val1 = val0;
            key0 = key; val0 = val;
          }
          *cell = val0;
        }
        if (bound_flags) {
          const uint32_t pend = __ballot((raise & 4u) != 0) ? 4u : 0u, zero = __ballot((raise & 8u) != 0) ? 8u : 0u;
          if ((pend | zero) && lane == 0) atomicOr(bound_flags, pend | zero);
        }
        __syncthreads();
      }
      constexpr int kQuads = kTileRows / 4;
      for (int it = tid; it < n_pass * kQuads; it += kCompatThreads) {
        const int al = it / kQuads, r0 = 4 * (it % kQuads);
        const double* const cell = &tile[al * kTileLd + r0];
        double v[4];
#pragma unroll
        for (int j = 0; j < 4; ++j) v[j] = cell[j];
        if (r0 < n_r) {
          double* const dst = probs + (int64_t)(a_base + al) * n_rows + row0 + r0;
          if (r0 + 4 <= n_r) {
#pragma unroll
            for (int j = 0; j < 4; ++j) dst[j] = v[j];
          } else {
#pragma unroll
            for (int j = 0; j < 4; ++j)
              if (r0 + j < n_r) dst[j] = v[j];
          }
        }
        if (kLog && miss8) {
          uint32_t packed = 0;
#pragma unroll
          for (int j = 0; j < 4; ++j) {
            if (r0 + j < n_r) {
              const double t = __builtin_fma(v[j], -1.0 / 3.0, 0.25);
              uint32_t m;
              if (t < 100.0) m = (uint32_t)(int)t;
              else { m = 255u; if (v[j] == v[j]) atomicOr(bound_flags, 1u); }
              packed |= m << (8 * j);
            }
          }
          *reinterpret_cast<uint32_t*>(miss8 + (int64_t)(a_base + al) * ldm + row0 + r0) = packed;
        }
      }
    }
    if (kLog && miss8 && tile_i == n_tiles - 1) {
      const int64_t pad0 = n_tiles * kTileRows;
      const int n_pad = (int)((ldm - pad0) / 4);
      for (int it = tid; it < n_pass * n_pad; it += kCompatThreads) {
        const int al = it / n_pad, w = it % n_pad;
        *reinterpret_cast<uint32_t*>(miss8 + (int64_t)(a_base + al) * ldm + pad0 + 4 * w) = 0u;
      }
    }
    __syncthreads();
  }
}

__global__ __launch_bounds__(kThreads) void patch_pending(double* __restrict__ L, int64_t n_rows, int n_allele,
                                                          LutView lut, uint8_t* __restrict__ miss8, int64_t ldm,
                                                          uint32_t* __restrict__ flags) {
  const int64_t n = n_rows * (int64_t)n_allele;
  const int64_t stride = (int64_t)gridDim.x * kThreads;
  uint64_t key0 = kLutEmptyKey;
  double val0 = 0.0;
  bool ok0 = false;
  for (int64_t i = (int64_t)blockIdx.x * kThreads + threadIdx.x; i < n; i += stride) {
    const double v = L[i];
    if (!(v > 0.0)) continue;
    const uint64_t key = (uint64_t)__double_as_longlong(v);
    if (key != key0) {
      key0 = key;
      val0 = gk_lut_lookup(lut, key, &ok0);
    }
    if (!ok0) { atomicOr(flags, 4u); continue; }
    L[i] = val0;
    const uint32_t m = gk_miss_of_log(val0);
    if (m == 255u && val0 == val0) atomicOr(flags, 1u);
    const int64_t a = i / n_rows, r = i - a * n_rows;
    miss8[a * ldm + r] = (uint8_t)m;
  }
}

template <bool kLog>
int launch_compat(gk_ctx* ctx, gk_tab* tab, gk_dptr d_rows, int64_t n_rows, gk_dptr d_vflag, int vbeg, int vend,
                  gk_dptr d_mask, int words, int n_allele, double* out, uint8_t* miss, uint16_t* nvar, LutView view,
                  int keep_empty, uint8_t* miss8 = nullptr, int64_t ldm = 0, uint32_t* bound_flags = nullptr,
                  uint16_t* lidx = nullptr, const int32_t* table_cols = nullptr, int n_table_cols = 0) {
  const double empty_p = keep_empty ? 0.999 : 1.0;
  const int words_in = words;
  int32_t* d_cols = nullptr;
  if (n_table_cols > 0) {
    n_allele = n_table_cols;
    words = (n_table_cols + 31) / 32;
    GK_HIP(gk_pool_malloc(ctx, (void**)&d_cols, (size_t)n_table_cols * sizeof(int32_t)));
    if (gk_send(ctx, d_cols, table_cols, (size_t)n_table_cols * sizeof(int32_t)) != hipSuccess) {
      gk_pool_free(ctx, d_cols);
      gk_set_error("compatibility table: sending the column list failed: %s", hipGetErrorString(hipGetLastError()));
      return GK_ERR_HIP;
    }
  }
  int64_t want = ((n_rows + kTileRows - 1) / kTileRows + 7) / 8 * 8;
  const dim3 grid((unsigned)(want < 2048 ? (want < 8 ? 8 : want) : 2048)), block(kCompatThreads);
  const int64_t n_mask = (int64_t)(vend - vbeg) * words;
  uint32_t* mask_t = nullptr;
  if (gk_pool_malloc(ctx, (void**)&mask_t, (size_t)std::max<int64_t>(n_mask, 1) * sizeof(uint32_t)) != hipSuccess) {
    gk_pool_free(ctx, d_cols);
    gk_set_error("out of device memory for the transposed bit matrix");
    return GK_ERR_HIP;
  }
  if (n_mask > 0 && d_cols)
    GK_KERNEL(transpose_gather_mask, dim3((unsigned)((n_mask + kThreads - 1) / kThreads)), dim3(kThreads), 0, ctx->stream,
              gk_ptr<uint32_t>(d_mask), vend - vbeg, words_in, d_cols, n_table_cols, words, mask_t, bound_flags);
  else if (n_mask > 0)
    GK_KERNEL(transpose_mask, dim3((unsigned)((n_mask + kThreads - 1) / kThreads)), dim3(kThreads), 0, ctx->stream,
              gk_ptr<uint32_t>(d_mask), vend - vbeg, words, mask_t, bound_flags);
  else if (bound_flags)
    GK_HIP(hipMemsetAsync(bound_flags, 0, sizeof(uint32_t), ctx->stream));
  for (int a_base = 0; a_base < n_allele; a_base += 64 * kMaxSlots) {
    const int slots = std::min(kMaxSlots, (n_allele - a_base + 63) / 64);
#define GK_COMPAT_GO(S, IDX)                                                                                        \
  GK_KERNEL((compat_kernel<kLog, S, !kLog, IDX>), grid, block, 0, ctx->stream, gk_ptr<int32_t>(d_rows), n_rows,     \
            tab->d_off, tab->d_ids, gk_ptr<uint8_t>(d_vflag), vbeg, vend, mask_t, words, n_allele, a_base, out,     \
            miss, nvar, view, empty_p, miss8, ldm, bound_flags, lidx)
#define GK_COMPAT_LAUNCH(S)                              \
  GK_PROF(ctx, "compat_kernel", {                        \
    if (kLog && lidx) GK_COMPAT_GO(S, (kLog && true));   \
    else GK_COMPAT_GO(S, false);                         \
  })
    switch (slots) {
      case 1: GK_COMPAT_LAUNCH(1); break;
      case 2: GK_COMPAT_LAUNCH(2); break;
      case 3: GK_COMPAT_LAUNCH(3); break;
      default: GK_COMPAT_LAUNCH(4); break;
    }
#undef GK_COMPAT_LAUNCH
#undef GK_COMPAT_GO
  }
  gk_pool_free(ctx, mask_t);
  gk_pool_free(ctx, d_cols);
  GK_HIP(hipGetLastError());
  return GK_OK;
}

}

extern "C" {

static int build_partition(gk_ctx* ctx, gk_tab* tab, int multiple) {
  gk_tab::GenePartition& part = tab->part[multiple ? 1 : 0];
  const int64_t n = tab->n_valid;
  const int n_bins = tab->idx ? tab->idx->n_gene : 256;
  const int64_t n_tiles = (n + 63) / 64;
  const size_t n_hist = (size_t)n_bins * n_tiles;
  uint32_t *hist = nullptr, *goff = nullptr;
  GK_HIP(gk_pool_malloc(ctx, (void**)&hist, (n_hist + 1) * sizeof(uint32_t)));
  GK_HIP(gk_pool_malloc(ctx, (void**)&goff, (size_t)(n_bins + 1) * sizeof(uint32_t)));
  GK_HIP(gk_pool_malloc(ctx, (void**)&part.d_rows, (size_t)(n + 1) * sizeof(int32_t)));
  part.owner = ctx;
  GK_HIP(hipMemsetAsync(hist, 0, n_hist * sizeof(uint32_t), ctx->stream));
  GK_PROF(ctx, "part_pass", GK_KERNEL(part_pass<false>, dim3(nblk(n)), dim3(kThreads), 0, ctx->stream,
                                               tab->d_pair_gene, tab->d_pair_nh, n, multiple, n_bins, n_tiles, hist,
                                               (int32_t*)nullptr));
  int rc = gk_scan_u32(ctx, hist, (int64_t)n_hist, hist + n_hist);
  if (rc) return rc;
  GK_PROF(ctx, "part_pass", GK_KERNEL(part_pass<true>, dim3(nblk(n)), dim3(kThreads), 0, ctx->stream,
                                               tab->d_pair_gene, tab->d_pair_nh, n, multiple, n_bins, n_tiles, hist,
                                               part.d_rows));
  GK_KERNEL(part_offsets, dim3((unsigned)(n_bins / 256 + 1)), dim3(256), 0, ctx->stream, hist, hist + n_hist,
                     n_bins, n_tiles, goff);
  GK_HIP(hipGetLastError());
  std::vector<uint32_t> host((size_t)n_bins + 1);
  GK_HIP(gk_fetch(ctx, host.data(), goff, host.size() * sizeof(uint32_t)));
  part.gene_off.assign(host.begin(), host.end());
  gk_pool_free(ctx, hist);
  gk_pool_free(ctx, goff);
  return GK_OK;
}

int gk_select_gene(gk_ctx* ctx, gk_tab* tab, int gene, int multiple, gk_dptr d_rows_out, int64_t* n_out) {
  gk_bind(ctx);
  GK_REQUIRE(ctx && tab && n_out, "null pointer");
  *n_out = 0;
  if (tab->n_valid == 0 || gene < 0) return GK_OK;
  gk_tab::GenePartition& part = tab->part[multiple ? 1 : 0];
  {
    std::lock_guard<std::mutex> lock(tab->part_mutex);
    if (part.gene_off.empty()) {
      int rc = build_partition(ctx, tab, multiple);
      if (rc) { part.gene_off.clear(); return rc; }
    }
  }
  if ((size_t)gene + 1 >= part.gene_off.size()) return GK_OK;
  const int64_t first = part.gene_off[gene], count = part.gene_off[gene + 1] - first;
  if (count > 0) {
    GK_REQUIRE(d_rows_out, "null output");
    GK_HIP(hipMemcpyAsync(gk_ptr<int32_t>(d_rows_out), part.d_rows + first, (size_t)count * sizeof(int32_t),
                          hipMemcpyDeviceToDevice, ctx->stream));
  }
  *n_out = count;
  return GK_OK;
}

int gk_select_nonempty(gk_ctx* ctx, gk_tab* tab, gk_dptr d_rows, int64_t n_rows, gk_dptr d_vflag, gk_dptr d_rows_out,
                       int64_t* n_out) {
  gk_bind(ctx);
  GK_REQUIRE(ctx && tab && n_out, "null pointer");
  if (n_rows == 0) { *n_out = 0; return GK_OK; }
  uint32_t* flag = nullptr;
  GK_HIP(gk_pool_malloc(ctx, (void**)&flag, (size_t)n_rows * sizeof(uint32_t)));
  GK_PROF(ctx, "flag_nonempty", GK_KERNEL(flag_nonempty, dim3(nblk(n_rows)), dim3(kThreads), 0, ctx->stream, gk_ptr<int32_t>(d_rows),
                     n_rows, tab->d_off, tab->d_ids, gk_ptr<uint8_t>(d_vflag), flag, (uint32_t*)nullptr, 0));
  int rc = gk_compact(ctx, flag, gk_ptr<int32_t>(d_rows), n_rows, gk_ptr<int32_t>(d_rows_out), n_out);
  gk_pool_free(ctx,flag);
  return rc;
}

int gk_variant_count_range(gk_ctx* ctx, gk_tab* tab, gk_dptr d_rows, int64_t n_rows, gk_dptr d_vflag, gk_dptr d_cnt,
                            int32_t vbeg, int32_t vend);
// ... 48 lines not shown
    if (!mine) { flag[v] = 0; return; }
  }
  const uint8_t f = vflag[v];
  flag[v] = ((!(f & 1) && cnt_pos[v]) || (!(f & 2) && cnt_neg[v])) ? 1u : 0u;
}
__global__ __launch_bounds__(kThreads) void gather_surviving(const int32_t* ord, int64_t n, const uint32_t* cnt_pos,
                                                             const uint32_t* cnt_neg, const uint8_t* vflag,
                                                             uint32_t* out ) {
  const int64_t i = (int64_t)blockIdx.x * kThreads + threadIdx.x;
  if (i >= n) return;
  const int32_t v = ord[i];
  const uint8_t f = vflag[v];
  out[i] = (f & 1) ? 0u : cnt_pos[v];
  out[n + i] = (f & 2) ? 0u : cnt_neg[v];
}
__global__ __launch_bounds__(kThreads) void gather_surviving_queued(const int32_t* ord, const uint32_t* d_n, int64_t cap,
                                                                    const uint32_t* cnt_pos, const uint32_t* cnt_neg,
                                                                    const uint8_t* vflag, uint32_t* out ) {
  const int64_t i = (int64_t)blockIdx.x * kThreads + threadIdx.x;
  if (i >= cap || i >= (int64_t)*d_n) return;
  const int32_t v = ord[i];
  const uint8_t f = vflag[v];
  out[i] = (f & 1) ? 0u : cnt_pos[v];
  out[cap + i] = (f & 2) ? 0u : cnt_neg[v];
}
}

static int variant_surviving(gk_ctx* ctx, gk_tab* tab, gk_dptr d_cnt, gk_dptr d_vflag, int64_t max_out, int32_t* ord_out,
                             uint32_t* pos_out, uint32_t* neg_out, int64_t* n_out, int gene, int vbeg, int vend) {
  gk_bind(ctx);
  GK_REQUIRE(ctx && tab && ord_out && pos_out && neg_out && n_out, "null pointer");
  const int64_t nv = (int64_t)tab->n_var + tab->n_novel;
  *n_out = 0;
  if (!nv) return GK_OK;
  uint32_t* cnt = gk_ptr<uint32_t>(d_cnt);
  uint32_t *flag = nullptr, *vals = nullptr;
  int32_t* ord = nullptr;
  GK_HIP(gk_pool_malloc(ctx, (void**)&flag, (size_t)nv * sizeof(uint32_t)));
  GK_HIP(gk_pool_malloc(ctx, (void**)&ord, (size_t)nv * sizeof(int32_t)));
  GK_KERNEL(flag_surviving, dim3(nblk(nv)), dim3(kThreads), 0, ctx->stream, cnt, cnt + nv,
                     gk_ptr<uint8_t>(d_vflag), nv, flag, gene, vbeg, vend, tab->n_var, tab->d_novel_key);
  int64_t n = 0;
  int rc = gk_compact(ctx, flag, nullptr, nv, ord, &n);
  if (rc == GK_OK && n > max_out) {
    gk_set_error("surviving-variant buffer too small (%lld > %lld)", (long long)n, (long long)max_out);
    rc = GK_ERR_CAPACITY;
  }
  if (rc == GK_OK && n) {
    GK_HIP(gk_pool_malloc(ctx, (void**)&vals, (size_t)(2 * n) * sizeof(uint32_t)));
    GK_KERNEL(gather_surviving, dim3(nblk(n)), dim3(kThreads), 0, ctx->stream, ord, n, cnt, cnt + nv,
                       gk_ptr<uint8_t>(d_vflag), vals);
    GK_HIP(gk_fetch_queue(ctx, ord_out, ord, (size_t)n * sizeof(int32_t)));
    GK_HIP(gk_fetch_queue(ctx, pos_out, vals, (size_t)n * sizeof(uint32_t)));
    GK_HIP(gk_fetch_queue(ctx, neg_out, vals + n, (size_t)n * sizeof(uint32_t)));
    GK_HIP(gk_fetch_wait(ctx));
    gk_pool_free(ctx, vals);
  }
  gk_pool_free(ctx, flag);
  gk_pool_free(ctx, ord);
  if (rc == GK_OK) *n_out = n;
  return rc;
}

int gk_variant_surviving(gk_ctx* ctx, gk_tab* tab, gk_dptr d_cnt, gk_dptr d_vflag, int64_t max_out, int32_t* ord_out,
                         uint32_t* pos_out, uint32_t* neg_out, int64_t* n_out) {
  return variant_surviving(ctx, tab, d_cnt, d_vflag, max_out, ord_out, pos_out, neg_out, n_out, -1, 0, 0);
}

int gk_variant_surviving_gene(gk_ctx* ctx, gk_tab* tab, gk_dptr d_cnt, gk_dptr d_vflag, int32_t gene, int32_t vbeg,
                              int32_t vend, int64_t max_out, int32_t* ord_out, uint32_t* pos_out, uint32_t* neg_out,
                              int64_t* n_out) {
  GK_REQUIRE(gene >= 0 && vend >= vbeg, "bad gene range");
  return variant_surviving(ctx, tab, d_cnt, d_vflag, max_out, ord_out, pos_out, neg_out, n_out, gene, vbeg, vend);
}

namespace {
struct Survivors {
  int64_t max_out = 0;
  int32_t* ord = nullptr;
  uint32_t *pos = nullptr, *neg = nullptr;
  int64_t* n_out = nullptr;
  uint64_t* novel_key = nullptr;
};
}

static int sample_prepare(gk_ctx* ctx, gk_tab* tab, int32_t multiple, gk_dptr d_vflag, gk_dptr d_cnt, gk_dptr d_rows,
                          int64_t* gene_off_out, const Survivors* surv, bool keep_vflag = false, int rounds = 1,
                          gk_dptr d_cnt_full = 0);

int gk_sample_prepare(gk_ctx* ctx, gk_tab* tab, int32_t multiple, gk_dptr d_vflag, gk_dptr d_cnt, gk_dptr d_rows,
                      int64_t* gene_off_out) {
  return sample_prepare(ctx, tab, multiple, d_vflag, d_cnt, d_rows, gene_off_out, nullptr);
}

int gk_sample_prepare_all(gk_ctx* ctx, gk_tab* tab, int32_t multiple, gk_dptr d_vflag, gk_dptr d_cnt, gk_dptr d_rows,
                          int64_t* gene_off_out, int64_t max_out, int32_t* ord_out, uint32_t* pos_out, uint32_t* neg_out,
                          int64_t* n_out, uint64_t* novel_key_out) {
  GK_REQUIRE(ord_out && pos_out && neg_out && n_out && max_out >= 0, "null pointer");
  Survivors s;
  s.max_out = max_out; s.ord = ord_out; s.pos = pos_out; s.neg = neg_out; s.n_out = n_out; s.novel_key = novel_key_out;
  return sample_prepare(ctx, tab, multiple, d_vflag, d_cnt, d_rows, gene_off_out, &s);
}

int gk_sample_prepare_exon(gk_ctx* ctx, gk_tab* tab, int32_t multiple, gk_dptr d_vflag, gk_dptr d_cnt, gk_dptr d_rows,
                           int64_t* gene_off_out, int64_t max_out, int32_t* ord_out, uint32_t* pos_out, uint32_t* neg_out,
                           int64_t* n_out) {
  GK_REQUIRE(ord_out && pos_out && neg_out && n_out && max_out >= 0, "null pointer");
  Survivors s;
  s.max_out = max_out; s.ord = ord_out; s.pos = pos_out; s.neg = neg_out; s.n_out = n_out; s.novel_key = nullptr;
  return sample_prepare(ctx, tab, multiple, d_vflag, d_cnt, d_rows, gene_off_out, &s, true, 2);
}

int gk_sample_prepare_exon_from(gk_ctx* ctx, gk_tab* tab, int32_t multiple, gk_dptr d_vflag, gk_dptr d_cnt, gk_dptr d_rows,
                                int64_t* gene_off_out, int64_t max_out, int32_t* ord_out, uint32_t* pos_out,
                                uint32_t* neg_out, int64_t* n_out, gk_dptr d_cnt_full) {
  GK_REQUIRE(ord_out && pos_out && neg_out && n_out && max_out >= 0, "null pointer");
  GK_REQUIRE(d_cnt_full != d_cnt || !d_cnt, "the full model's tallies and the exon model's are two buffers");
  Survivors s;
  s.max_out = max_out; s.ord = ord_out; s.pos = pos_out; s.neg = neg_out; s.n_out = n_out; s.novel_key = nullptr;
  return sample_prepare(ctx, tab, multiple, d_vflag, d_cnt, d_rows, gene_off_out, &s, true, 2, d_cnt_full);
}

static int sample_prepare(gk_ctx* ctx, gk_tab* tab, int32_t multiple, gk_dptr d_vflag, gk_dptr d_cnt, gk_dptr d_rows,
                          int64_t* gene_off_out, const Survivors* surv, bool keep_vflag, int rounds, gk_dptr d_cnt_full) {
  gk_bind(ctx);
  GK_REQUIRE(ctx && tab && tab->idx && d_vflag && d_cnt && d_rows && gene_off_out, "null pointer");
  if (surv) *surv->n_out = 0;
  const int n_gene = tab->idx->n_gene;
  const int64_t nv = (int64_t)tab->n_var + tab->n_novel;
  hipStream_t st = ctx->stream;
  for (int g = 0; g <= n_gene; ++g) gene_off_out[g] = 0;
  if (!keep_vflag) GK_HIP(hipMemsetAsync(gk_ptr<void>(d_vflag), 0, (size_t)std::max<int64_t>(nv, 1), st));
  GK_HIP(hipMemsetAsync(gk_ptr<void>(d_cnt), 0, (size_t)std::max<int64_t>(2 * nv, 1) * sizeof(uint32_t), st));
  auto novel_only = [&]() -> int {
    if (surv && surv->novel_key && tab->n_novel > 0)
      GK_HIP(gk_fetch(ctx, surv->novel_key, tab->d_novel_key, (size_t)tab->n_novel * sizeof(uint64_t)));
    return GK_OK;
  };
  if (tab->n_valid == 0) return novel_only();
  gk_tab::GenePartition& part = tab->part[multiple ? 1 : 0];
  {
    std::lock_guard<std::mutex> lock(tab->part_mutex);
    if (part.gene_off.empty()) {
      int rc = build_partition(ctx, tab, multiple);
      if (rc) { part.gene_off.clear(); return rc; }
    }
  }
  GK_REQUIRE((int)part.gene_off.size() >= n_gene + 1, "partition does not cover the genes");
  const int64_t n_rows = part.gene_off[n_gene];
  if (n_rows == 0) return novel_only();
  std::vector<int32_t> wg_gene;
  std::vector<int64_t> wg_row0, wg_row1, goff(part.gene_off.begin(), part.gene_off.begin() + n_gene + 1);
  const int64_t per_wg = std::max<int64_t>(64, (n_rows + 2047) / 2048);
  int max_span = 0;
  for (int g = 0; g < n_gene; ++g) {
    max_span = std::max(max_span, tab->idx->gene_vbeg[g + 1] - tab->idx->gene_vbeg[g]);
    for (int64_t r = goff[g]; r < goff[g + 1]; r += per_wg) {
      wg_gene.push_back(g);
      wg_row0.push_back(r);
      wg_row1.push_back(std::min(goff[g + 1], r + per_wg));
    }
  }
  const int max_local = std::min(max_span, 60 * 1024 / 8);
  const size_t n_wg = wg_gene.size();
  char* d_tab = nullptr;
  const size_t o_row0 = (n_wg * sizeof(int32_t) + 15) / 16 * 16, o_row1 = o_row0 + n_wg * sizeof(int64_t),
               o_goff = o_row1 + n_wg * sizeof(int64_t), tab_bytes = o_goff + (size_t)(n_gene + 1) * sizeof(int64_t);
  {
    std::vector<char> packed(tab_bytes);
    memcpy(packed.data(), wg_gene.data(), n_wg * sizeof(int32_t));
    memcpy(packed.data() + o_row0, wg_row0.data(), n_wg * sizeof(int64_t));
    memcpy(packed.data() + o_row1, wg_row1.data(), n_wg * sizeof(int64_t));
    memcpy(packed.data() + o_goff, goff.data(), (size_t)(n_gene + 1) * sizeof(int64_t));
    GK_HIP(gk_pool_malloc(ctx, (void**)&d_tab, tab_bytes));
    GK_HIP(gk_send(ctx, d_tab, packed.data(), tab_bytes));
  }
  uint32_t* cnt = gk_ptr<uint32_t>(d_cnt);
  uint8_t* vflag = gk_ptr<uint8_t>(d_vflag);
  uint8_t *maybe = nullptr, *alive = nullptr;
  GK_HIP(gk_pool_malloc(ctx, (void**)&maybe, (size_t)tab->n_valid));
  GK_HIP(gk_pool_malloc(ctx, (void**)&alive, (size_t)tab->n_valid));
  GK_HIP(hipMemsetAsync(maybe, 0, (size_t)tab->n_valid, st));
  for (int round = 0; round < rounds; ++round) {
    if (round) GK_HIP(hipMemsetAsync(cnt, 0, (size_t)(2 * nv) * sizeof(uint32_t), st));
    if (round == 0 && rounds > 1 && d_cnt_full) {
      const uint32_t* full = gk_ptr<const uint32_t>(d_cnt_full);
      GK_PROF(ctx, "mask_tallies", GK_KERNEL(mask_tallies, dim3(nblk(nv)), dim3(kThreads), 0, st, full, full + nv, vflag, nv, cnt, cnt + nv));
    } else {
      GK_PROF(ctx, "count_ids_genes",
              GK_KERNEL(count_ids_genes, dim3((unsigned)n_wg), dim3(kThreads), (size_t)max_local * 8 + kThreads * sizeof(uint32_t), st, part.d_rows,
                        (const int32_t*)d_tab, (const int64_t*)(d_tab + o_row0), (const int64_t*)(d_tab + o_row1),
                        tab->idx->d_gene_vbeg, max_local, tab->d_off, tab->d_ids, vflag, cnt, cnt + nv,
                        round == rounds - 1 ? maybe : (uint8_t*)nullptr));
    }
    GK_PROF(ctx, "apply_correction", GK_KERNEL(apply_correction, dim3(nblk(nv)), dim3(kThreads), 0, st, cnt, cnt + nv, nv, vflag));
  }
  uint32_t *flag = nullptr, *kept = nullptr;
  GK_HIP(gk_pool_malloc(ctx, (void**)&flag, (size_t)n_rows * sizeof(uint32_t)));
  GK_HIP(gk_pool_malloc(ctx, (void**)&kept, (size_t)n_gene * sizeof(uint32_t)));
  GK_PROF(ctx, "flag_pairs", GK_KERNEL(flag_pairs, dim3(nblk(4 * (int64_t)tab->n_valid)), dim3(kThreads), 0, st, (int64_t)tab->n_valid,
                                   tab->d_off, tab->d_ids, vflag, maybe, alive));
  GK_PROF(ctx, "gather_pair_flags", GK_KERNEL(gather_pair_flags, dim3(nblk(std::max<int64_t>(n_rows, n_gene))), dim3(kThreads), 0, st,
                                          part.d_rows, n_rows, alive, flag, kept, n_gene));
  GK_PROF(ctx, "count_flags_per_gene", GK_KERNEL(count_flags_per_gene, dim3((unsigned)n_gene, kFlagSlices), dim3(kThreads), 0, st, flag,
                                      (const int64_t*)(d_tab + o_goff), kept));
  GK_HIP(hipGetLastError());
  std::vector<void*> temps{flag, kept, d_tab, alive, maybe};
  auto done = [&](int code) {
    for (void* t : temps) gk_pool_free(ctx, t);
    return code;
  };
  uint32_t* d_total = nullptr;
  int rc = gk_compact_enqueue(ctx, flag, part.d_rows, n_rows, gk_ptr<int32_t>(d_rows), &d_total, temps);
  if (rc) return done(rc);
  uint32_t total = 0, n_surv = 0;
  std::vector<uint32_t> host((size_t)n_gene);
  bool queued = gk_fetch_queue(ctx, &total, d_total, sizeof(uint32_t)) == hipSuccess &&
                gk_fetch_queue(ctx, host.data(), kept, (size_t)n_gene * sizeof(uint32_t)) == hipSuccess;
  if (queued && surv && nv > 0) {
    const int64_t cap = std::min<int64_t>(nv, surv->max_out);
    uint32_t *sflag = nullptr, *vals = nullptr, *d_n = nullptr;
    int32_t* ord = nullptr;
    auto take = [&](void** p, size_t bytes) {
      if (gk_pool_malloc(ctx, p, bytes) != hipSuccess) return false;
      temps.push_back(*p);
      return true;
    };
    if (!take((void**)&sflag, (size_t)nv * sizeof(uint32_t)) || !take((void**)&ord, (size_t)nv * sizeof(int32_t)) ||
        !take((void**)&vals, (size_t)std::max<int64_t>(2 * cap, 1) * sizeof(uint32_t))) {
      gk_fetch_cancel(ctx);
      gk_set_error("out of device memory for the surviving tallies");
      return done(GK_ERR_HIP);
    }
    GK_KERNEL(flag_surviving, dim3(nblk(nv)), dim3(kThreads), 0, st, cnt, cnt + nv, vflag, nv, sflag, -1, 0, 0, tab->n_var,
              tab->d_novel_key);
    rc = gk_compact_enqueue(ctx, sflag, nullptr, nv, ord, &d_n, temps);
    if (rc) { gk_fetch_cancel(ctx); return done(rc); }
    if (cap > 0) {
      GK_KERNEL(gather_surviving_queued, dim3(nblk(cap)), dim3(kThreads), 0, st, ord, d_n, cap, cnt, cnt + nv, vflag, vals);
      queued = gk_fetch_queue(ctx, surv->ord, ord, (size_t)cap * sizeof(int32_t)) == hipSuccess &&
               gk_fetch_queue(ctx, surv->pos, vals, (size_t)cap * sizeof(uint32_t)) == hipSuccess &&
               gk_fetch_queue(ctx, surv->neg, vals + cap, (size_t)cap * sizeof(uint32_t)) == hipSuccess;
    }
    queued = queued && gk_fetch_queue(ctx, &n_surv, d_n, sizeof(uint32_t)) == hipSuccess;
    if (queued && surv->novel_key && tab->n_novel > 0)
      queued = gk_fetch_queue(ctx, surv->novel_key, tab->d_novel_key, (size_t)tab->n_novel * sizeof(uint64_t)) == hipSuccess;
  }
  if (!queued || gk_fetch_wait(ctx) != hipSuccess) {
    gk_fetch_cancel(ctx);
    gk_set_error("sample preamble: %s", hipGetErrorString(hipGetLastError()));
    return done(GK_ERR_HIP);
  }
  int64_t run = 0;
  for (int g = 0; g < n_gene; ++g) { gene_off_out[g] = run; run += host[g]; }
  gene_off_out[n_gene] = run;
  if (run != (int64_t)total) { gk_set_error("non-empty rows per gene do not add up"); return done(GK_ERR_ASSERT); }
  if (surv) {
    if ((int64_t)n_surv > surv->max_out) {
      gk_set_error("surviving-variant buffer too small (%lld > %lld)", (long long)n_surv, (long long)surv->max_out);
      return done(GK_ERR_CAPACITY);
    }
    *surv->n_out = n_surv;
  }
  return done(GK_OK);
}

int gk_compat(gk_ctx* ctx, gk_tab* tab, gk_dptr d_rows, int64_t n_rows, gk_dptr d_vflag, int32_t vbeg, int32_t vend,
              gk_dptr d_mask, int32_t words, int32_t n_allele, int32_t keep_empty, gk_dptr d_probs, gk_dptr d_miss,
              gk_dptr d_nvar) {
  gk_bind(ctx);
  GK_REQUIRE(ctx && tab, "null pointer");
  GK_REQUIRE(words >= 1 && n_allele >= 0 && n_allele <= words * 32 && vend >= vbeg, "bad mask geometry");
  if (n_rows == 0 || n_allele == 0) return GK_OK;
  return launch_compat<false>(ctx, tab, d_rows, n_rows, d_vflag, vbeg, vend, d_mask, words, n_allele,
                              gk_ptr<double>(d_probs), gk_ptr<uint8_t>(d_miss), gk_ptr<uint16_t>(d_nvar), LutView{}, keep_empty);
}

int gk_compat_log(gk_ctx* ctx, gk_tab* tab, gk_dptr d_rows, int64_t n_rows, gk_dptr d_vflag, int32_t vbeg,
                  int32_t vend, gk_dptr d_mask, int32_t words, int32_t n_allele, int32_t keep_empty, gk_lut* lut,
                  gk_dptr d_log) {
  gk_bind(ctx);
  GK_REQUIRE(ctx && tab && lut, "null pointer");
  GK_REQUIRE(words >= 1 && n_allele >= 0 && n_allele <= words * 32 && vend >= vbeg, "bad mask geometry");
  if (n_rows == 0 || n_allele == 0) return GK_OK;
  GK_REQUIRE(d_log, "null output");
  return launch_compat<true>(ctx, tab, d_rows, n_rows, d_vflag, vbeg, vend, d_mask, words, n_allele,
                             gk_ptr<double>(d_log), nullptr, nullptr, gk_lut_view(lut), keep_empty);
}

int gk_compat_log_miss(gk_ctx* ctx, gk_tab* tab, gk_dptr d_rows, int64_t n_rows, gk_dptr d_vflag, int32_t vbeg,
                       int32_t vend, gk_dptr d_mask, int32_t words, int32_t n_allele, int32_t keep_empty, gk_lut* lut,
                       gk_dptr d_log, gk_dptr d_miss8, int64_t ldm, gk_dptr d_flags) {
  gk_bind(ctx);
  GK_REQUIRE(ctx && tab && lut, "null pointer");
  GK_REQUIRE(words >= 1 && n_allele >= 0 && n_allele <= words * 32 && vend >= vbeg, "bad mask geometry");
  if (n_rows == 0 || n_allele == 0) return GK_OK;
  GK_REQUIRE(d_log && d_miss8 && d_flags, "null output");
  GK_REQUIRE(ldm >= n_rows && ldm % 64 == 0, "mismatch table stride must be a multiple of 64 rows");
  return launch_compat<true>(ctx, tab, d_rows, n_rows, d_vflag, vbeg, vend, d_mask, words, n_allele,
                             gk_ptr<double>(d_log), nullptr, nullptr, gk_lut_view(lut), keep_empty,
                             gk_ptr<uint8_t>(d_miss8), ldm, gk_ptr<uint32_t>(d_flags));
}

int gk_compat_log_miss_cols(gk_ctx* ctx, gk_tab* tab, gk_dptr d_rows, int64_t n_rows, gk_dptr d_vflag, int32_t vbeg,
                            int32_t vend, gk_dptr d_mask, int32_t words, int32_t n_allele, int32_t keep_empty, gk_lut* lut,
                            const int32_t* table_cols, int32_t n_table_cols, gk_dptr d_log, gk_dptr d_miss8, int64_t ldm,
                            gk_dptr d_flags) {
  gk_bind(ctx);
  GK_REQUIRE(ctx && tab && lut, "null pointer");
  GK_REQUIRE(words >= 1 && n_allele >= 0 && n_allele <= words * 32 && vend >= vbeg, "bad mask geometry");
  GK_REQUIRE(table_cols && n_table_cols >= 1 && n_table_cols <= n_allele, "bad column list");
  for (int c = 0; c < n_table_cols; ++c)
    GK_REQUIRE(table_cols[c] >= 0 && table_cols[c] < n_allele && (c == 0 || table_cols[c] > table_cols[c - 1]),
               "table columns must be allele ordinals, ascending and unique");
  if (n_rows == 0) return GK_OK;
  GK_REQUIRE(d_log && d_miss8 && d_flags, "null output");
  GK_REQUIRE(ldm >= n_rows && ldm % 64 == 0, "mismatch table stride must be a multiple of 64 rows");
  return launch_compat<true>(ctx, tab, d_rows, n_rows, d_vflag, vbeg, vend, d_mask, words, n_allele,
                             gk_ptr<double>(d_log), nullptr, nullptr, gk_lut_view(lut), keep_empty,
                             gk_ptr<uint8_t>(d_miss8), ldm, gk_ptr<uint32_t>(d_flags), nullptr, table_cols, n_table_cols);
}

int gk_compat_patch(gk_ctx* ctx, gk_lut* lut, gk_dptr d_log, int64_t n_rows, int32_t n_allele, gk_dptr d_miss8, int64_t ldm,
                    gk_dptr d_flags) {
  gk_bind(ctx);
  GK_REQUIRE(ctx && lut && d_log && d_miss8 && d_flags && n_rows >= 0 && n_allele >= 0 && ldm >= n_rows, "bad patch arguments");
  GK_HIP(hipMemsetAsync(gk_ptr<void>(d_flags), 0, sizeof(uint32_t), ctx->stream));
  if (n_rows == 0 || n_allele == 0) return GK_OK;
  const int64_t n = n_rows * (int64_t)n_allele;
  const int64_t want = (n + kThreads - 1) / kThreads;
  GK_PROF(ctx, "patch_pending",
          GK_KERNEL(patch_pending, dim3((unsigned)(want < 4096 ? want : 4096)), dim3(kThreads), 0, ctx->stream,
                    gk_ptr<double>(d_log), n_rows, n_allele, gk_lut_view(lut), gk_ptr<uint8_t>(d_miss8), ldm,
                    gk_ptr<uint32_t>(d_flags)));
  GK_HIP(hipGetLastError());
  return GK_OK;
}

int gk_compat_index(gk_ctx* ctx, gk_tab* tab, gk_dptr d_rows, int64_t n_rows, gk_dptr d_vflag, int32_t vbeg, int32_t vend,
                    gk_dptr d_mask, int32_t words, int32_t n_allele, int32_t keep_empty, gk_lut* lut, gk_dptr d_lidx,
                    gk_dptr d_miss8, int64_t ldm, gk_dptr d_flags) {
  gk_bind(ctx);
  GK_REQUIRE(ctx && tab && lut, "null pointer");
  GK_REQUIRE(words >= 1 && n_allele >= 0 && n_allele <= words * 32 && vend >= vbeg, "bad mask geometry");
  if (n_rows == 0 || n_allele == 0) return GK_OK;
  GK_REQUIRE(d_lidx && d_miss8 && d_flags, "null output");
  GK_REQUIRE(ldm >= n_rows && ldm % 64 == 0, "table stride must be a multiple of 64 rows");
  return launch_compat<true>(ctx, tab, d_rows, n_rows, d_vflag, vbeg, vend, d_mask, words, n_allele, nullptr, nullptr,
                             nullptr, gk_lut_view(lut), keep_empty, gk_ptr<uint8_t>(d_miss8), ldm,
                             gk_ptr<uint32_t>(d_flags), gk_ptr<uint16_t>(d_lidx));
}

}
```

kir_graph_amd/engine.py:

```python
from __future__ import annotations

import ctypes as C
import os
import threading
from typing import NamedTuple

import numpy as np

from . import _lib
from ._lib import Device, DeviceBuffer, DeviceSlice, TabInfo, check, lib
from .index import GkIndex, KEY_POS_SHIFT, KEY_TYP_SHIFT, KEY_VAL_MASK
from .msa2hisat import Variant

TYPE_OF_RANK = {0: "insertion", 1: "single", 2: "deletion"}


def _i32(a) -> np.ndarray:
    return np.ascontiguousarray(a, dtype=np.int32)


def searchMode() -> str:
    mode = os.environ.get("GK_SEARCH", "bound")
    if mode not in ("bound", "exact"):
        raise ValueError(f"GK_SEARCH={mode!r}: expected 'bound' or 'exact'")
    return mode


class Surviving(NamedTuple):
    ordinals: np.ndarray
    pos: np.ndarray
    neg: np.ndarray
    bounds: np.ndarray

    def ofGene(self, g: int) -> tuple[np.ndarray, np.ndarray, np.ndarray]:
        a, b = int(self.bounds[g]), int(self.bounds[g + 1])
        return self.ordinals[a:b], self.pos[a:b], self.neg[a:b]


class PreparedGene(NamedTuple):
    rows: DeviceBuffer
    n_rows: int
    vflag: DeviceBuffer
    tally: DeviceBuffer
    tally_gene: tuple[int, int, int]
    surviving: tuple[np.ndarray, np.ndarray, np.ndarray] | None = None


class PreparedSample(NamedTuple):
    vflag: DeviceBuffer
    cnt: DeviceBuffer
    rows: DeviceBuffer
    off: np.ndarray
    surviving: Surviving

    def gene(self, g: int, vbeg: int, vend: int, dev: Device | None = None) -> PreparedGene:
        a, b = int(self.off[g]), int(self.off[g + 1])
        return PreparedGene(DeviceSlice(self.rows, a, b - a, dev), b - a, self.vflag, self.cnt, (g, vbeg, vend),
                            self.surviving.ofGene(g))


def _groupByGene(gene_of: np.ndarray, o: np.ndarray, p: np.ndarray, q: np.ndarray, n_genes: int) -> Surviving:
    order = np.argsort(gene_of, kind="stable")
    bounds = np.searchsorted(gene_of[order], np.arange(n_genes + 1)).astype(np.int64)
    return Surviving(np.ascontiguousarray(o[order], dtype=np.int32), np.ascontiguousarray(p[order], dtype=np.uint32),
                     np.ascontiguousarray(q[order], dtype=np.uint32), bounds)


class DeviceIndex:

    def __init__(self, dev: Device, index: GkIndex):
        self.dev, self.host = dev, index
        h = C.c_void_p()
        key = np.ascontiguousarray(index.key, dtype=np.uint64)
        vbeg = _i32(index.gene_vbeg)
        check(lib().gk_index_create(dev.ctx, key.ctypes.data, len(key), vbeg.ctypes.data, len(index.genes),
                                    C.byref(h)))
        self.handle = h
        self.masks = [dev.put(t.mask) for t in index.tables]

    def close(self) -> None:
        if self.handle:
            lib().gk_index_destroy(self.handle)
            self.handle = None


class Tabulation:

    def __init__(self, dindex: DeviceIndex, mates, novel_base: int = 0, dev: Device | None = None,
                 correction: tuple[np.ndarray, np.ndarray] | None = None,
                 spill: tuple[np.ndarray, np.ndarray] | None = None):
        self.dev, self.dindex = dev or dindex.dev, dindex
        self._spill, self._correction = spill, correction
        if isinstance(mates, np.ndarray):
            assert mates.dtype == _lib.MATE_DTYPE
            self.mates = self.dev.put(mates)
        elif hasattr(mates, "toDevice"):
            self.mates = mates.toDevice(self.dev)
        else:
            self.mates = mates
        self.n_pairs = self.mates.size // 2
        compact = getattr(self.mates, "words", None) if hasattr(self.mates, "records") else None
        h = C.c_void_p()
        d_table = d_pos0 = None
        if correction is not None:
            table, pos0 = correction
            assert table.dtype == np.uint8 and table.shape == (int(pos0[-1]), 5) and len(pos0) == len(dindex.host.genes) + 1
            d_table = self.dev.put(np.ascontiguousarray(table).reshape(-1) if table.size else np.zeros(1, np.uint8))
            d_pos0 = self.dev.put(np.ascontiguousarray(pos0, dtype=np.int64))
        wide = which = None
        if spill is not None and len(spill[1]):
            wide = np.ascontiguousarray(spill[0], dtype=_lib.MATE_WIDE_DTYPE)
            which = np.ascontiguousarray(spill[1], dtype=np.int64)
            assert len(wide) == 2 * len(which)
        if compact is not None:
            check(lib().gk_tabulate_compact(self.dev.ctx, dindex.handle, compact.ptr, self.n_pairs,
                                            d_table.ptr if d_table else 0, d_pos0.ptr if d_pos0 else 0,
                                            wide.ctypes.data if wide is not None else None,
                                            which.ctypes.data if which is not None else None,
                                            len(which) if which is not None else 0, C.byref(h)))
        elif wide is not None:
            check(lib().gk_tabulate_spilled(self.dev.ctx, dindex.handle, self.mates.ptr, self.n_pairs,
                                            d_table.ptr if d_table else 0, d_pos0.ptr if d_pos0 else 0,
                                            wide.ctypes.data, which.ctypes.data, len(which), C.byref(h)))
        elif correction is None:
            check(lib().gk_tabulate(self.dev.ctx, dindex.handle, self.mates.ptr, self.n_pairs, C.byref(h)))
        else:
            check(lib().gk_tabulate_corrected(self.dev.ctx, dindex.handle, self.mates.ptr, self.n_pairs,
                                              d_table.ptr, d_pos0.ptr, C.byref(h)))
        self.handle = h
        info = TabInfo()
        check(lib().gk_tab_get_info(h, C.byref(info)))
        self.info = info
        self.n_valid, self.n_ids, self.n_novel = int(info.n_valid), int(info.n_ids), int(info.n_novel)
        self.novel_base = novel_base
        if info.err_flags & 1:
            raise AssertionError("variant window has left > right (graphkir/hisat2.py:744)")
        self._novel_keys = None
        if self.dev.call_log is not None:
            self.dev.call_log.append(("tab_count", self.n_pairs, self.n_valid, self.n_ids)
                                     + ((compact.nbytes,) if compact is not None else ()))

    @property
    def n_var_total(self) -> int:
        override = getattr(self, "_id_names", None)
        if override is not None:
            return len(override)
        return self.dindex.host.n_variant + self.n_novel

    def close(self) -> None:
        if self.handle and not getattr(self, "_borrowed", False):
            for prep in (getattr(self, "_prepared", None) or {}).values():
                for b in (prep.vflag, prep.cnt, prep.rows):
                    b.free()
            self._prepared = {}
            lib().gk_tab_destroy(self.handle)
        self.handle = None

    def prepared(self, dev: Device, multiple: bool = False, exon: bool = False) -> PreparedSample | None:
        if self.dindex is None or not self.info.d_pair_src:
            return None
        root = getattr(self, "_root", self)
        lock = root.__dict__.setdefault("_prep_lock", threading.Lock())
        store = root.__dict__.setdefault("_prepared", {})
        key = (bool(multiple), True) if exon else bool(multiple)
        with lock:
            prep = store.get(key)
            if prep is None:
                host = self.dindex.host
                nv = max(self.n_var_total, 1)
                if exon:
                    flags = np.full(nv, 3, dtype=np.uint8)
                    flags[:host.n_variant][host.in_exon.astype(bool)] = 0
                    vflag = dev.put(flags)
                else:
                    vflag = dev.alloc(nv, np.uint8)
                cnt = dev.alloc(2 * nv, np.uint32)
                rows = dev.alloc(max(self.n_valid, 1), np.int32)
                off = np.zeros(len(host.genes) + 1, dtype=np.int64)
                o, p, q = (np.empty(nv, dtype=t) for t in (np.int32, np.uint32, np.uint32))
                n_surv = C.c_int64()
                args = (dev.ctx, self.handle, int(multiple), vflag.ptr, cnt.ptr, rows.ptr, off.ctypes.data, nv,
                        o.ctypes.data, p.ctypes.data, q.ctypes.data, C.byref(n_surv))
                if exon:
                    full = store.get(bool(multiple))
                    if full is not None:
                        check(lib().gk_sample_prepare_exon_from(*args, full.cnt.ptr))
                    else:
                        check(lib().gk_sample_prepare_exon(*args))
                else:
                    want_novel = self._novel_keys is None and self.n_novel > 0
                    novel_keys = np.empty(self.n_novel, dtype=np.uint64) if want_novel else None
                    check(lib().gk_sample_prepare_all(*args, novel_keys.ctypes.data if want_novel else None))
                    if want_novel:
                        self._novel_keys = root._novel_keys = novel_keys
                o, p, q = o[:n_surv.value], p[:n_surv.value], q[:n_surv.value]
                gene_of = np.searchsorted(host.gene_vbeg, o, side="right") - 1
                if not exon and len(o) and int(o[-1]) >= host.n_variant:
                    is_novel = o >= host.n_variant
                    gene_of[is_novel] = (self.novelKeys()[o[is_novel] - host.n_variant] >> np.uint64(56)).astype(gene_of.dtype)
                prep = store[key] = PreparedSample(vflag, cnt, rows, off, _groupByGene(gene_of, o, p, q, len(host.genes)))
        return prep

    @staticmethod
    def survivingOfGene(prep: PreparedSample, g: int):
        return prep.surviving.ofGene(g)

    def on(self, dev: Device) -> "Tabulation":
        if dev is self.dev:
            return self
        import copy
        other = copy.copy(self)
        other.dev = dev
        other._borrowed = True
        other._root = getattr(self, "_root", self)
        return other

    def offsets(self) -> np.ndarray:
        return self.dev.view(self.info.d_off, 4 * self.n_valid + 1, np.uint32)

    def ids(self) -> np.ndarray:
        return self.dev.view(self.info.d_ids, self.n_ids, np.uint32)

    def pairSrc(self) -> np.ndarray:
        return self.dev.view(self.info.d_pair_src, self.n_valid, np.int32)

    def pairGene(self) -> np.ndarray:
        return self.dev.view(self.info.d_pair_gene, self.n_valid, np.uint8)

    def pairNH(self) -> np.ndarray:
        return self.dev.view(self.info.d_pair_nh, self.n_valid, np.uint8)

    def novelKeys(self) -> np.ndarray:
        if self._novel_keys is None:
            self._novel_keys = self.dev.view(self.info.d_novel_key, self.n_novel, np.uint64)
        return self._novel_keys

    def novelVariants(self, ins_strings: list[str]) -> list[Variant]:
        genes = self.dindex.host.genes
        out = []
        for rank, k in enumerate(self.novelKeys().tolist()):
            ref = genes[k >> 56]
            pos = (k >> KEY_POS_SHIFT) & 0xFFFFFF
            typ = TYPE_OF_RANK[(k >> KEY_TYP_SHIFT) & 3]
            val = k & KEY_VAL_MASK
            if typ == "single":
                v = Variant(pos=pos, typ=typ, ref=ref, val=chr(val), length=1)
            elif typ == "deletion":
                v = Variant(pos=pos, typ=typ, ref=ref, val=int(val), length=int(val))
            else:
                s = ins_strings[val]
                v = Variant(pos=pos, typ=typ, ref=ref, val=s, length=len(s))
            v.id = f"nv{self.novel_base + rank}"
            out.append(v)
        return out

    def idNames(self) -> list[str]:
        override = getattr(self, "_id_names", None)
        if override is not None:
            return override
        names = [str(v.id) for v in self.dindex.host.variants]
        names += [f"nv{self.novel_base + r}" for r in range(self.n_novel)]
        self._id_names = names
        return names

    def labelTables(self):
        if getattr(self, "_variant_src", None) is not None:
            return None
        root = getattr(self, "_root", self)
        tables = root.__dict__.get("_label_tables")
        if tables is None:
            keys_all = np.ascontiguousarray(np.concatenate([self.dindex.host.key, self.novelKeys()]), dtype=np.uint64)
            strings = getattr(self, "ins_strings", None) or self.dindex.host.ins_strings
            ins_code = np.array([ord(s) if len(s) == 1 else 256 + i for i, s in enumerate(strings)] or [0], dtype=np.int64)
            tables = root.__dict__["_label_tables"] = (keys_all, ins_code)
        return tables

    def labelCodes(self, ordinals):
        if getattr(self, "_variant_src", None) is not None:
            return None
        keys_all = getattr(self, "_keys_all", None)
        if keys_all is None:
            keys_all = self._keys_all = np.concatenate([self.dindex.host.key, self.novelKeys()])
        k = keys_all[np.asarray(ordinals, dtype=np.int64)].astype(np.int64)
# ... 382 lines not shown
```

kir_graph_amd/kir_typing.py:

```python
from __future__ import annotations

import contextlib
import ctypes as C
import json
import os
import sys
import threading
import time
from typing import Any

import numpy as np

from . import _lib
from ._lib import Device
from .call_bootstrap import MAX_BOOT, MAX_TOP, CallBootstrap, bootstrapCall, homoFactor
from .call_coverage import CallCoverage, coverCall
from .call_fit import MAX_EXTRA, CallFit, fitCall
from .engine import PreparedGene, PreparedSample, searchMode
from .hisat2 import SampleData, loadCompact, loadReadsAndVariantsData
from .typing_em import (EmBootstrap, Hisat2AlleleResult, bootstrapEM, callsByAbundance, candidateSetsDistinct,
                        hisat2TypingPerGene, summariseBootstrap)
from .typing_mulit_allele import (AlleleTyping, AlleleTypingExonFirst, ReadSet, StepList, isHetrozygous,
                                  sharedLogTable)
from .utils import NumpyEncoder, logger, testHook, traceOn
# ... 121 lines not shown
        flags = np.full(tab.n_var_total, 3, dtype=np.uint8)
        flags[:idx.n_variant][idx.in_exon.astype(bool)] = 0
        return flags


class _OnLane(Typing):

    def __init__(self) -> None:
        super().__init__()
        self._local = threading.local()
        self.slot_base = 0
        self.tables_rewritten = 0
        self.tables_patched = 0

    def _context(self):
        tab = getattr(self._local, "tab", None)
        if tab is None:
            base = self._data.tab
            dev = base.dev.worker(self.slot_base)
            tab = self._local.tab = base.on(dev)
            self._local.logs = sharedLogTable(dev)
        return tab, self._local.logs


_SEARCH_SLOTS: dict = {}
_SEARCH_SLOTS_LOCK = threading.Lock()


def _searchSlot():
    n = int(os.environ.get("GK_SEARCH_SLOTS", "0") or 0)
    if n <= 0:
        return contextlib.nullcontext()
    with _SEARCH_SLOTS_LOCK:
        sem = _SEARCH_SLOTS.get(n)
        if sem is None:
            sem = _SEARCH_SLOTS[n] = threading.BoundedSemaphore(n)
    return sem


class TypingWithPosNegAllele(_OnLane):

    def __init__(self, filename_variant_json, top_n: int = 300, multiple: bool = False, exon_first: bool = False,
                 exon_only: bool = False, exon_candidate_threshold: float = .9, variant_correction: bool = False,
                 device: Device | None = None, call_bootstrap: int = 0, call_bootstrap_seed: int = 2022,
                 call_bootstrap_top: int = 32, call_fit: bool = False, call_fit_extra: int = 3,
                 call_coverage: bool = False, call_coverage_len: dict[str, int] | None = None):
        super().__init__()
        if call_coverage and not call_coverage_len:
            raise ValueError("call_coverage: needs call_coverage_len, the backbone length of every gene")
        self._call_coverage = (bool(call_coverage), dict(call_coverage_len or {}))
        self.call_coverage: dict[str, CallCoverage | None] = {}
        if not 0 <= int(call_fit_extra) <= MAX_EXTRA:
            raise ValueError(f"call_fit_extra: the extra alleles listed must lie in 0 .. {MAX_EXTRA}")
        self._call_fit = (bool(call_fit), int(call_fit_extra))
        self.call_fit: dict[str, CallFit] = {}
        if not 0 <= int(call_bootstrap) <= MAX_BOOT:
            raise ValueError(f"call_bootstrap: the number of replicates must lie in 0 .. {MAX_BOOT}")
        if not 1 <= int(call_bootstrap_top) <= MAX_TOP:
            raise ValueError(f"call_bootstrap_top: the candidate sets kept must lie in 1 .. {MAX_TOP}")
        self._call_boot = (int(call_bootstrap), int(call_bootstrap_seed), int(call_bootstrap_top))
        self.call_bootstrap: dict[str, CallBootstrap] = {}
        self._data = _sample(filename_variant_json, device)
        self._multiple = multiple
        self._top_n = top_n
        self._exon_first, self._exon_only = exon_first, exon_only
        self._exon_candidate_threshold = exon_candidate_threshold
        self._variant_correction = variant_correction

    def typing(self, gene_cn: dict[str, int], min_reads_num: int = 100) -> tuple[list[str], list[str]]:
        if self._wholeSample():
            return self._typingWholeSample(gene_cn, min_reads_num)
        if self._wholeSampleExonFirst():
            return self._typingWholeSampleExonFirst(gene_cn, min_reads_num)
        return super().typing(gene_cn, min_reads_num)

    def _wholeSampleExonFirst(self) -> bool:
        return (self._exon_first and not self._exon_only and os.environ.get("GK_INDEX_TABLE", "0") != "1"
                and searchMode() == "bound")

    def _typingWholeSampleExonFirst(self, gene_cn: dict[str, int], min_reads_num: int) -> tuple[list[str], list[str]]:
        full_tables = testHook("full_tables") is not None
        tab, logs = self._context()
        udev = tab.dev.urgent()
        prep_f = tab.prepared(udev, self._multiple)
        if prep_f is None:
            return super().typing(gene_cn, min_reads_num)
        prep_e = tab.prepared(udev, self._multiple, exon=True)
        top_n, threshold = self._top_n, self._exon_candidate_threshold
        todo = [(gene, int(cn)) for gene, cn in gene_cn.items() if cn]
        views = [_GeneView(self._data, gene, self._multiple, tab=tab) for gene, _ in todo]
        verd_e = self._zygosityVerdicts(tab, prep_e, [(v.g, cn) for v, (_, cn) in zip(views, todo)])

        plan: dict[int, dict] = {}
        jobs1 = []
        for k, ((gene, cn), view) in enumerate(zip(todo, views)):
            if view.g is None or not view.alleles:
                continue
            prepared_e, prepared_f = view.prepared(prep_e), view.prepared(prep_f)
            if prepared_e.n_rows == 0 or prepared_f.n_rows == 0:
                continue
            allele_group, grouped, group_names, exon_mask = AlleleTypingExonFirst.exonGroups(
                view.variants, view.n_span, view.groupCache(), tab.dev)
            force = False if isHetrozygous(gene) else None
            typ_e = view.model(logs, prepared_e, variants=grouped, mask=exon_mask, alleles=group_names, force_homo=force,
                               top_n=top_n, variant_correction=True, _defer_launch=True)
            job, homo = typ_e.geneJob(cn, verd_e.get(view.g) if cn > 1 else False)
            plan[k] = {"typ_e": typ_e, "homo_e": homo, "job1": len(jobs1), "groups": allele_group,
                       "full": prepared_f, "force": force}
            jobs1.append(job)
        self.tables_rewritten = self.tables_patched = 0
        self.exon_info: dict[str, dict] = {}
        if jobs1:
            with self._searchBatch(tab, logs, prep_e.vflag, jobs1) as (jobs, handles):
                for k, p in plan.items():
                    q = p["job1"]
                    p["typ_e"].adoptJob(jobs[q], C.c_void_p(handles[q]), todo[k][1], p["homo_e"])
        jobs2, keep_alive = [], []
        for k, p in plan.items():
            (gene, cn), view = todo[k], views[k]
            result = p["typ_e"].result[-1]
            result.setNameGroup(p["groups"])

            def full_model(table_cols=None):
                return view.model(logs, p["full"], force_homo=p["force"], top_n=top_n // 5, variant_correction=True,
                                  _defer_launch=True, _table_cols=table_cols)
            if not result.value.shape[0]:
                logger.warning("[Allele] Cannot typing with exon-only reads. Typing with exon+intron")
                p["full_model"] = full_model()
                p["fallback"] = True
                continue
            ranks = list(result.topRank(threshold=threshold))
            self.exon_info[gene] = {"exon_groups": len(p["groups"]), "exon_sets": int(result.value.shape[0]),
                                    "candidates": len(ranks)}
            if len(ranks) > 1024:
                p["per_gene"] = True
                continue
            allele_to_id = {a: i for i, a in enumerate(view.alleles)}
            cand_steps = [[np.ascontiguousarray([allele_to_id[a] for a in names], dtype=np.int32)
                           for names in result.allele_name_group[i]] for i in ranks]
            table_cols = np.unique(np.concatenate([c for steps in cand_steps for c in steps])).astype(np.int32)
            if full_tables or len(table_cols) == len(view.alleles):
                table_cols = None
            full = p["full_model"] = full_model(table_cols)
            self.exon_info[gene]["table_columns"] = len(view.alleles) if table_cols is None else len(table_cols)
            job, _ = full.geneJob(cn, False)
            job.n_steps = 0
            p["job2"] = len(jobs2)
            jobs2.append(job)
            p["cands"] = []
            for steps in cand_steps:
                cols = np.ascontiguousarray(np.concatenate(steps), dtype=np.int32)
                offs = np.ascontiguousarray(np.concatenate([[0], np.cumsum([len(x) for x in steps])]), dtype=np.int32)
                keep_alive += [cols, offs]
                cand = _lib.GeneJob(d_rows=job.d_rows, n_rows=job.n_rows, d_mask=job.d_mask, d_L=0, d_miss8=0, ldm=job.ldm,
                                    d_msum=0, d_flags=0, d_lidx=0, vbeg=job.vbeg, vend=job.vend, words=job.words,
                                    n_allele=job.n_allele, n_steps=len(steps), top_n=top_n // 5, bound_ok=0, passes=0,
                                    indexed=0, patches=0, table_of=p["job2"], n_step_cols=len(steps),
                                    step_cols=cols.ctypes.data, step_cols_off=offs.ctypes.data)
                p["cands"].append((len(jobs2), len(steps)))
                jobs2.append(cand)
        if jobs2:
            with self._searchBatch(tab, logs, prep_f.vflag, jobs2) as (jobs, handles):
                for k, p in plan.items():
                    if "job2" not in p:
                        continue
                    full = p["full_model"]
                    full.adoptTable(jobs[p["job2"]], C.c_void_p(handles[p["job2"]]))
# ... 320 lines not shown
```

kir_graph_amd/roofmodel.py:

```python
from __future__ import annotations

HBM_PEAK_GBS = 8000.0
TILE = 32
N_SIMD = 256 * 4
NOMINAL_HZ = 2.4e9

ISSUE_CYCLES = {"v_mul_f64": 4.50, "v_add_f64": 4.26, "v_max_f64": 4.19, "v_bfe_i32": 4.43, "v_bfi_b32": 4.56,
                "v_sad_u8": 4.49}
GUIDE_CYCLES = {"v_mul_f64": 4.0, "v_add_f64": 4.0, "v_max_f64": 4.0, "v_bfe_i32": 2.0, "v_bfi_b32": 2.0, "v_sad_u8": 2.0}
SEQUENCE_CYCLES = {"compat_kernel": 5.81}
KERNEL_OPS = {
    "compat_kernel": ("v_bfe_i32", "v_bfi_b32", "v_bfi_b32", "v_mul_f64"),
    "minsum_sad": ("v_sad_u8",),
    "maxsum_chunks": ("v_max_f64", "v_add_f64"),
}


def laneOpsPeak(kernel: str, table: dict[str, float] = ISSUE_CYCLES) -> float:
    ops = KERNEL_OPS[kernel]
    return len(ops) * 64 * N_SIMD * NOMINAL_HZ / sum(table[o] for o in ops)


def symmetricOutputs(n: int) -> int:
    total = 0
    for t0 in range(0, n, TILE):
        rows = min(TILE, n - t0)
        total += rows * (n - t0)
    return total


def maxsumLaunch(n_rows: int, n_sets: int, c_prev: int, n_cols: int, n_prev_cols: int,
                 symmetric: bool = False) -> tuple[float, float]:
    by = 8.0 * n_rows * (n_cols + n_prev_cols) + 8.0 * n_sets * n_cols
    outputs = symmetricOutputs(n_cols) if symmetric else n_sets * n_cols
    return by, 2.0 * n_rows * outputs


def minsumLaunch(n_rows: int, n_sets: int, n_cols: int, n_prev_cols: int, symmetric: bool = False
                 ) -> tuple[float, float]:
    outputs = symmetricOutputs(n_cols) if symmetric else n_sets * n_cols
    return 1.0 * n_rows * (n_cols + n_prev_cols) + 4.0 * n_sets * n_cols, n_rows * outputs / 4.0


def compatLaunch(n_rows: int, n_allele: int, n_ids: float, out_bytes: int = 8) -> tuple[float, float]:
    return 4.0 * n_ids + 16.0 * n_rows + float(out_bytes + 1) * n_rows * n_allele, 4.0 * n_ids * n_allele


def tabLaunch(n_pairs: int, n_valid: int, n_ids: int, record_bytes: float | None = None) -> tuple[float, float]:
    read = 256.0 * n_pairs if record_bytes is None else float(record_bytes)
    return read + 4.0 * n_ids + 22.0 * n_valid, 0.0


def setsumLaunch(n_rows: int, n_sets: int, c: int, n_distinct: int) -> tuple[float, float]:
    return 8.0 * n_rows * n_distinct + 8.0 * n_sets * (c + 1), float(n_rows) * n_sets * (c + 1)


def emSetsLaunch(n_rows: int, n_ids: float, set_words: int) -> tuple[float, float]:
    return 24.0 * n_rows + 4.0 * n_ids + 4.0 * set_words, 0.0


def emVerifyLaunch(set_words: int) -> tuple[float, float]:
    return 4.0 * set_words, 0.0


def _priced(kernel: str, calls: list[tuple]) -> tuple[float, float, str, float]:
    by = ops = 0.0
    bound, peak = "hbm", 0.0
    for c in calls:
        if kernel == "maxsum_chunks":
            b, o = maxsumLaunch(*c[1:7])
            bound, peak = "valu", laneOpsPeak("maxsum_chunks")
        elif kernel == "colsum_chunks":
            b, o = 8.0 * c[1] * c[4] + 8.0 * c[4], 0.0
        elif kernel == "em_sets_groups":
            b, o = emSetsLaunch(*c[1:4])
        elif kernel == "em_sets_verify":
            b, o = emVerifyLaunch(c[3])
        elif kernel == "minsum_sad":
            b, o = minsumLaunch(*c[1:6])
            bound, peak = "valu", laneOpsPeak("minsum_sad")
        elif kernel == "compat_kernel":
            b, o = compatLaunch(*c[1:5])
            bound, peak = "valu", laneOpsPeak("compat_kernel")
        elif kernel == "compat_rows8":
            b, o = compatLaunch(*c[1:5])[0], 0.0
        elif kernel == "tab_count":
            b, o = tabLaunch(*c[1:5])
        elif kernel in ("fraction_chunks", "setsum_leaves"):
            b, o = setsumLaunch(*c[1:5])
        else:
            return 0.0, 0.0, "hbm", 0.0
        by += b
        ops += o
    return by, ops, bound, peak


def summarise(call_log: list[tuple], kernel: str, total_ms: float, launches: int) -> dict:
    calls = [c for c in call_log if c[0] == kernel]
    base = {"kernel": kernel, "bound": "hbm", "achieved": None, "peak": HBM_PEAK_GBS, "unit": "GB/s",
            "frac": None, "traffic": None, "launches": launches, "avg_launch_ms": total_ms / max(launches, 1)}
    if not calls or total_ms <= 0:
        return base
    by, ops, bound, peak = _priced(kernel, calls)
    if by <= 0:
        return base
    sec = total_ms / 1e3
    gbs = by / sec / 1e9
    hbm = {"achieved": gbs, "peak": HBM_PEAK_GBS, "unit": "GB/s", "frac": gbs / HBM_PEAK_GBS}
    out = dict(base)
    out["algorithmic_bytes_per_launch"] = by / max(launches, 1)
    if bound == "valu":
        tops = ops / sec / 1e12
        unit = {"maxsum_chunks": "Tops/s f64 (max+add)", "minsum_sad": "T lane-ops/s (v_sad_u8, 4 reads each)",
                "compat_kernel": "T lane-ops/s (4 VALU per id and allele)"}.get(kernel, "T lane-ops/s")
        guide = laneOpsPeak(kernel, GUIDE_CYCLES)
        out.update({"bound": "valu", "achieved": tops, "peak": peak / 1e12, "unit": unit, "frac": ops / sec / peak,
                    "peak_guide": guide / 1e12, "frac_guide": ops / sec / guide,
                    "issue_cycles": {o: ISSUE_CYCLES[o] for o in KERNEL_OPS[kernel]},
                    "algorithmic_ops_per_launch": ops / max(launches, 1), "hbm": hbm,
                    "note": "VALU-issue bound (ordered f64 products / a (max,+) or (min,+) contraction).  `peak` = the "
                            "kernel's own instruction mix issued back to back at the MEASURED cost of each instruction "
                            "(tools/valu_rate.hip at 8 waves per SIMD, profiles/r03_valu_rate.txt: cycles of a 2.4 GHz "
                            "clock per wave64 instruction and SIMD in `issue_cycles`); `peak_guide` / `frac_guide` price "
                            "the same mix at the guide's 2 cycles per 32-bit and 4 per float64 instruction.  The HBM "
                            "roof is shown beside it; symmetric launches are credited with the triangle of tiles they "
                            "compute"})
        if kernel in SEQUENCE_CYCLES:
            seq = 64 * N_SIMD * NOMINAL_HZ / SEQUENCE_CYCLES[kernel]
            out["peak_sequence"] = seq / 1e12
            out["frac_sequence"] = ops / sec / seq
            out["note"] += (".  `peak_sequence` / `frac_sequence`: the same instructions at the rate measured for them "
                            "as the sequence the kernel issues (eight independent chains per wave, 8 waves per SIMD)")
    else:
        out.update(hbm)
        out["bound"] = "hbm"
    return out


def dominant(prof: dict[str, tuple[int, float]], call_log: list[tuple]) -> dict:
    if not prof:
        return summarise([], "none", 0.0, 0)
    priced = {k: v for k, v in prof.items() if _priced(k, [c for c in call_log if c[0] == k])[0] > 0}
    top = max(prof.items(), key=lambda kv: kv[1][1])[0]
    name, (launches, total_ms) = max((priced or prof).items(), key=lambda kv: kv[1][1])
    out = summarise(call_log, name, total_ms, launches)
    total = sum(v[1] for v in prof.values())
    out["share_of_kernel_time"] = total_ms / total if total else None
    if top != name:
        out["largest_kernel_by_time"] = top
    others = {}
    for k, (n, ms) in prof.items():
        if k != name and ms > 0.02 * total:
            e = summarise(call_log, k, ms, n)
            if e.get("achieved") is not None:
                others[k] = {f: e[f] for f in ("bound", "achieved", "peak", "unit", "frac", "avg_launch_ms")}
    if others:
        out["other_kernels"] = others
    return out


def stepRoofline(call_log: list[tuple], steps: int, ms_per_step: float) -> dict:
    kernels = sorted({c[0] for c in call_log})
    total_bytes = hbm_floor = valu_floor = valu_floor_guide = 0.0
    per_kernel = {}
    for k in kernels:
        calls = [c for c in call_log if c[0] == k]
        by, ops, bound, peak = _priced(k, calls)
        if by <= 0:
            continue
        total_bytes += by
# ... 19 lines not shown
```

Measured before the change: 538.1 million.

## Fuse exon-membership walk into full prepare pass and fold miss column sums into compat

The full-sample prepare pass now also records, per read, whether any of its variant ids are exonic, using a second ballot and a two-bit maybe flag. The later exon prepare can then skip its own walk over read ids and reuse that flag together with the full counts. The compat kernel also gains a variant that accumulates mismatch column sums in shared memory and adds them to global memory with atomics, replacing the separate colsum launch for wide tables. This trades extra register and shared-memory pressure and atomic traffic for fewer full passes over the id arrays.

```diff
diff --git a/include/graphkir_hip.h b/include/graphkir_hip.h
--- a/include/graphkir_hip.h
+++ b/include/graphkir_hip.h
@@ -153,6 +153,13 @@
 int gk_sample_prepare_exon_from(gk_ctx* ctx, gk_tab* tab, int32_t multiple, gk_dptr d_vflag, gk_dptr d_cnt, gk_dptr d_rows,
                                 int64_t* gene_off_out, int64_t max_out, int32_t* ord_out, uint32_t* pos_out,
                                 uint32_t* neg_out, int64_t* n_out, gk_dptr d_cnt_full);
+int gk_sample_prepare_all_exon(gk_ctx* ctx, gk_tab* tab, int32_t multiple, gk_dptr d_vflag, gk_dptr d_cnt, gk_dptr d_rows,
+                               int64_t* gene_off_out, int64_t max_out, int32_t* ord_out, uint32_t* pos_out,
+                               uint32_t* neg_out, int64_t* n_out, uint64_t* novel_key_out, gk_dptr d_exon_flags,
+                               gk_dptr d_maybe_exon);
+int gk_sample_prepare_exon_nowalk(gk_ctx* ctx, gk_tab* tab, int32_t multiple, gk_dptr d_vflag, gk_dptr d_cnt, gk_dptr d_rows,
+                                  int64_t* gene_off_out, int64_t max_out, int32_t* ord_out, uint32_t* pos_out,
+                                  uint32_t* neg_out, int64_t* n_out, gk_dptr d_cnt_full, gk_dptr d_maybe_exon);
 
 int gk_compat(gk_ctx* ctx, gk_tab* tab, gk_dptr d_rows, int64_t n_rows, gk_dptr d_vflag,
               int32_t vbeg, int32_t vend, gk_dptr d_mask, int32_t words, int32_t n_allele, int32_t keep_empty,
@@ -199,6 +206,10 @@
                               int32_t vbeg, int32_t vend, gk_dptr d_mask, int32_t words, int32_t n_allele,
                               int32_t keep_empty, gk_lut* lut, const int32_t* table_cols, int32_t n_table_cols,
                               gk_dptr d_log, gk_dptr d_miss8, int64_t ldm, gk_dptr d_flags, gk_dptr d_msum);
+int gk_compat_log_miss_sums(gk_ctx* ctx, gk_tab* tab, gk_dptr d_rows, int64_t n_rows, gk_dptr d_vflag,
+                            int32_t vbeg, int32_t vend, gk_dptr d_mask, int32_t words, int32_t n_allele,
+                            int32_t keep_empty, gk_lut* lut, const int32_t* table_cols, int32_t n_table_cols,
+                            gk_dptr d_log, gk_dptr d_miss8, int64_t ldm, gk_dptr d_flags, gk_dptr d_msum);
 int gk_compat_patch(gk_ctx* ctx, gk_lut* lut, gk_dptr d_log, int64_t n_rows, int32_t n_allele, gk_dptr d_miss8,
                     int64_t ldm, gk_dptr d_flags);
 int gk_compat_index(gk_ctx* ctx, gk_tab* tab, gk_dptr d_rows, int64_t n_rows, gk_dptr d_vflag, int32_t vbeg,
diff --git a/kir_graph_amd/_lib.py b/kir_graph_amd/_lib.py
--- a/kir_graph_amd/_lib.py
+++ b/kir_graph_amd/_lib.py
@@ -201,6 +201,9 @@
     "gk_compat_log_miss_narrow": (C.c_int, [C.c_void_p, C.c_void_p, C.c_uint64, C.c_int64, C.c_uint64, C.c_int32, C.c_int32,
                                             C.c_uint64, C.c_int32, C.c_int32, C.c_int32, C.c_void_p, C.c_void_p, C.c_int32,
                                             C.c_uint64, C.c_uint64, C.c_int64, C.c_uint64, C.c_uint64]),
+    "gk_compat_log_miss_sums": (C.c_int, [C.c_void_p, C.c_void_p, C.c_uint64, C.c_int64, C.c_uint64, C.c_int32, C.c_int32,
+                                          C.c_uint64, C.c_int32, C.c_int32, C.c_int32, C.c_void_p, C.c_void_p, C.c_int32,
+                                          C.c_uint64, C.c_uint64, C.c_int64, C.c_uint64, C.c_uint64]),
     "gk_compat_log_miss": (C.c_int, [C.c_void_p, C.c_void_p, C.c_uint64, C.c_int64, C.c_uint64, C.c_int32, C.c_int32,
                                      C.c_uint64, C.c_int32, C.c_int32, C.c_int32, C.c_void_p, C.c_uint64, C.c_uint64,
                                      C.c_int64, C.c_uint64]),
@@ -226,6 +229,12 @@
                                          C.c_int64, C.c_void_p, C.c_void_p, C.c_void_p, C.POINTER(C.c_int64)]),
     "gk_sample_prepare_exon_from": (C.c_int, [C.c_void_p, C.c_void_p, C.c_int32, C.c_uint64, C.c_uint64, C.c_uint64, C.c_void_p,
                                               C.c_int64, C.c_void_p, C.c_void_p, C.c_void_p, C.POINTER(C.c_int64), C.c_uint64]),
+    "gk_sample_prepare_all_exon": (C.c_int, [C.c_void_p, C.c_void_p, C.c_int32, C.c_uint64, C.c_uint64, C.c_uint64, C.c_void_p,
+                                             C.c_int64, C.c_void_p, C.c_void_p, C.c_void_p, C.POINTER(C.c_int64), C.c_void_p,
+                                             C.c_uint64, C.c_uint64]),
+    "gk_sample_prepare_exon_nowalk": (C.c_int, [C.c_void_p, C.c_void_p, C.c_int32, C.c_uint64, C.c_uint64, C.c_uint64,
+                                                C.c_void_p, C.c_int64, C.c_void_p, C.c_void_p, C.c_void_p, C.POINTER(C.c_int64),
+                                                C.c_uint64, C.c_uint64]),
     "gk_sample_em": (C.c_int, [C.c_void_p, C.c_void_p, C.c_void_p, C.c_int32, C.c_int32, C.c_double, C.c_void_p, C.c_void_p]),
     "gk_mates_compact": (C.c_int, [C.c_void_p, C.c_uint64, C.c_int64, C.POINTER(C.c_uint64), C.POINTER(C.c_int64)]),
     "gk_mates_expand": (C.c_int, [C.c_void_p, C.c_uint64, C.c_int64, C.c_uint64]),
diff --git a/kir_graph_amd/csrc/gk_hostsearch.cpp b/kir_graph_amd/csrc/gk_hostsearch.cpp
--- a/kir_graph_amd/csrc/gk_hostsearch.cpp
+++ b/kir_graph_amd/csrc/gk_hostsearch.cpp
@@ -200,6 +200,11 @@
                                                     int32_t keep_empty, gk_lut* lut, const int32_t* table_cols,
                                                     int32_t n_table_cols, gk_dptr d_log, gk_dptr d_miss8, int64_t ldm,
                                                     gk_dptr d_flags, gk_dptr d_msum);
+__attribute__((weak)) int gk_compat_log_miss_sums(gk_ctx* ctx, gk_tab* tab, gk_dptr d_rows, int64_t n_rows, gk_dptr d_vflag,
+                                                  int32_t vbeg, int32_t vend, gk_dptr d_mask, int32_t words, int32_t n_allele,
+                                                  int32_t keep_empty, gk_lut* lut, const int32_t* table_cols,
+                                                  int32_t n_table_cols, gk_dptr d_log, gk_dptr d_miss8, int64_t ldm,
+                                                  gk_dptr d_flags, gk_dptr d_msum);
 int gk_miss_colsum(gk_ctx* ctx, gk_dptr d_miss8, int64_t ldm, int32_t n_cols, gk_dptr d_msum);
 int gk_compat_patch(gk_ctx* ctx, gk_lut* lut, gk_dptr d_log, int64_t n_rows, int32_t n_allele, gk_dptr d_miss8, int64_t ldm,
                     gk_dptr d_flags);
@@ -826,9 +831,15 @@
       j.passes++;
       sticky[i] = 0;
       static const bool wide_compat = gk_test_hook("wide_compat");
+      static const bool separate_colsum = gk_test_hook("separate_colsum");
       if (j.n_table_cols > 0 && j.n_table_cols <= 8 && gk_compat_log_miss_narrow && !wide_compat) {
         rc = gk_compat_log_miss_narrow(ctx, tab, j.d_rows, j.n_rows, d_vflag, j.vbeg, j.vend, j.d_mask, j.words, j.n_allele, 0,
                                        lut, j.table_cols, j.n_table_cols, j.d_L, j.d_miss8, j.ldm, j.d_flags, j.d_msum);
+        summed = true;
+      } else if (gk_compat_log_miss_sums && !separate_colsum) {
+        rc = gk_compat_log_miss_sums(ctx, tab, j.d_rows, j.n_rows, d_vflag, j.vbeg, j.vend, j.d_mask, j.words, j.n_allele, 0,
+                                     lut, j.n_table_cols > 0 ? j.table_cols : nullptr, j.n_table_cols, j.d_L, j.d_miss8,
+                                     j.ldm, j.d_flags, j.d_msum);
         summed = true;
       } else if (j.n_table_cols > 0)
         rc = gk_compat_log_miss_cols(ctx, tab, j.d_rows, j.n_rows, d_vflag, j.vbeg, j.vend, j.d_mask, j.words, j.n_allele, 0,
diff --git a/kir_graph_amd/csrc/gk_typing.hip b/kir_graph_amd/csrc/gk_typing.hip
--- a/kir_graph_amd/csrc/gk_typing.hip
+++ b/kir_graph_amd/csrc/gk_typing.hip
@@ -112,12 +112,13 @@
 
 __global__ __launch_bounds__(kThreads) void flag_pairs(int64_t n_pairs, const uint32_t* __restrict__ off,
                                                        const uint32_t* __restrict__ ids, const uint8_t* __restrict__ vflag,
-                                                       const uint8_t* __restrict__ maybe, uint8_t* __restrict__ alive) {
+                                                       const uint8_t* __restrict__ maybe, uint8_t bits,
+                                                       uint8_t* __restrict__ alive) {
   const int64_t t = (int64_t)blockIdx.x * kThreads + threadIdx.x;
   const int64_t p = t >> 2;
   const uint32_t l = (uint32_t)t & 3u;
   uint32_t b = 0, mid = 0, e = 0;
-  if (p < n_pairs && maybe[p]) { b = off[4 * p]; mid = off[4 * p + 2]; e = off[4 * p + 4]; }
+  if (p < n_pairs && (maybe[p] & bits)) { b = off[4 * p]; mid = off[4 * p + 2]; e = off[4 * p + 4]; }
   const int shift = (threadIdx.x & 63) & ~3;
   bool any = false;
   for (uint32_t k0 = b; k0 < e && !any; k0 += 4) {
@@ -136,6 +137,7 @@
   if (i < n_rows) flag[i] = alive[rows[i]];
 }
 
+template <bool kExon>
 __global__ __launch_bounds__(kThreads) void count_ids_genes(const int32_t* __restrict__ rows,
                                                             const int32_t* __restrict__ wg_gene,
                                                             const int64_t* __restrict__ wg_row0,
@@ -144,7 +146,9 @@
                                                             const uint32_t* __restrict__ off,
                                                             const uint32_t* __restrict__ ids,
                                                             const uint8_t* __restrict__ vflag, uint32_t* cnt_pos,
-                                                            uint32_t* cnt_neg, uint8_t* __restrict__ maybe) {
+                                                            uint32_t* cnt_neg, uint8_t* __restrict__ maybe,
+                                                            const uint8_t* __restrict__ xflag,
+                                                            uint8_t* __restrict__ maybe_exon) {
   extern __shared__ uint32_t hist[];
   const int g = wg_gene[blockIdx.x];
   const int vbeg = gene_vbeg[g];
@@ -176,6 +180,15 @@
     }
     return counted;
   };
+  auto in_exon = [&](uint32_t k0, const uint8_t (&x)[kDeep]) {
+    bool any = false;
+#pragma unroll
+    for (int j = 0; j < kDeep; ++j) {
+      const uint32_t k = k0 + kGroup * j;
+      any = any || (k < e && !(x[j] & (k < mid ? 1 : 2)));
+    }
+    return any;
+  };
   auto ids_of = [&](uint32_t k0, uint32_t (&v)[kDeep]) {
     const uint32_t last = e ? e - 1u : 0u;
 #pragma unroll
@@ -183,22 +196,36 @@
   };
   for (; i < r1; i += kStep) {
     uint32_t v[kDeep];
-    uint8_t f[kDeep];
+    uint8_t f[kDeep], x[kDeep];
     ids_of(b + lane, v);
     const int64_t next = row1;
     const uint32_t nb = off[4 * next], nmid = off[4 * next + 2], ne = off[4 * next + 4];
     row1 = row_at(i + 2 * kStep);
 #pragma unroll
-    for (int j = 0; j < kDeep; ++j) f[j] = vflag[v[j]];
+    for (int j = 0; j < kDeep; ++j) {
+      if constexpr (kExon) { x[j] = xflag[v[j]]; f[j] = 0; }
+      else f[j] = vflag[v[j]];
+    }
     bool counted = tally(b + lane, v, f);
+    bool exonic = false;
+    if constexpr (kExon) exonic = in_exon(b + lane, x);
     for (uint32_t k0 = b + kGroup * kDeep + lane; k0 < e; k0 += kGroup * kDeep) {
       ids_of(k0, v);
 #pragma unroll
-      for (int j = 0; j < kDeep; ++j) f[j] = vflag[v[j]];
+      for (int j = 0; j < kDeep; ++j) {
+        if constexpr (kExon) { x[j] = xflag[v[j]]; f[j] = 0; }
+        else f[j] = vflag[v[j]];
+      }
       counted = tally(k0, v, f) || counted;
-    }
-    if (maybe) {
-      const bool any = ((__ballot(counted) >> ((threadIdx.x & 63) & ~(kGroup - 1))) & 0xFFFFull) != 0ull;
+      if constexpr (kExon) exonic = in_exon(k0, x) || exonic;
+    }
+    const int group_shift = (threadIdx.x & 63) & ~(kGroup - 1);
+    if constexpr (kExon) {
+      const bool any = ((__ballot(counted) >> group_shift) & 0xFFFFull) != 0ull;
+      const bool any_exon = ((__ballot(exonic) >> group_shift) & 0xFFFFull) != 0ull;
+      if (lane == 0) maybe_exon[row] = (uint8_t)((any ? 1 : 0) | (any_exon ? 2 : 0));
+    } else if (maybe) {
+      const bool any = ((__ballot(counted) >> group_shift) & 0xFFFFull) != 0ull;
       if (lane == 0) maybe[row] = any ? 1 : 0;
     }
     row = (int32_t)next;
@@ -239,9 +266,10 @@
 constexpr int kTileLd = kTileRows + 1;
 
 __global__ __launch_bounds__(kThreads) void transpose_mask(const uint32_t* mask, int n_span, int words, uint32_t* out,
-                                                           uint32_t* zero_word) {
+                                                           uint32_t* zero_word, uint32_t* zero_sums, int n_sums) {
   if (zero_word && blockIdx.x == 0 && threadIdx.x == 0) *zero_word = 0;
   const int64_t i = (int64_t)blockIdx.x * kThreads + threadIdx.x;
+  if (zero_sums) for (int64_t k = i; k < n_sums; k += (int64_t)gridDim.x * kThreads) zero_sums[k] = 0;
   if (i >= (int64_t)n_span * words) return;
   const int w = (int)(i / n_span), v = (int)(i % n_span);
   out[i] = mask[(int64_t)v * words + w];
@@ -250,9 +278,10 @@
 __global__ __launch_bounds__(kThreads) void transpose_gather_mask(const uint32_t* __restrict__ mask, int n_span, int words,
                                                                   const int32_t* __restrict__ cols, int n_cols,
                                                                   int words_out, uint32_t* __restrict__ out,
-                                                                  uint32_t* zero_word) {
+                                                                  uint32_t* zero_word, uint32_t* zero_sums, int n_sums) {
   if (zero_word && blockIdx.x == 0 && threadIdx.x == 0) *zero_word = 0;
   const int64_t i = (int64_t)blockIdx.x * kThreads + threadIdx.x;
+  if (zero_sums) for (int64_t k = i; k < n_sums; k += (int64_t)gridDim.x * kThreads) zero_sums[k] = 0;
   if (i >= (int64_t)n_span * words_out) return;
   const int w = (int)(i / n_span), v = (int)(i % n_span);
   const uint32_t* const row = mask + (int64_t)v * words;
@@ -267,18 +296,24 @@
 
 constexpr uint16_t kNoIndex = 0xFFFFu;
 
-template <bool kLog, int kSlots, bool kMiss, bool kIdx>
+template <bool kLog, int kSlots, bool kMiss, bool kIdx, bool kSum = false>
 __global__ __launch_bounds__(kCompatThreads) void compat_kernel(const int32_t* rows, int64_t n_rows, const uint32_t* off,
                                                                 const uint32_t* ids, const uint8_t* vflag, int vbeg, int vend,
                                                                 const uint32_t* mask_t, int words, int n_allele, int a_base,
                                                                 double* probs, uint8_t* miss_out, uint16_t* nvar_out,
                                                                 LutView lut, double empty_p, uint8_t* miss8, int64_t ldm,
-                                                                uint32_t* bound_flags, uint16_t* lidx) {
+                                                                uint32_t* bound_flags, uint16_t* lidx,
+                                                                uint32_t* msum) {
   const int n_span = vend - vbeg;
   constexpr int kPassAlleles = 64 * kSlots;
   constexpr int kPassWords = 2 * kSlots;
   __shared__ double tile[kPassAlleles * kTileLd];
   __shared__ uint32_t wave_rows[kCompatWaves][65 * kPassWords];
+  __shared__ uint32_t col_sum[kSum ? kPassAlleles : 1];
+  if (kSum) {
+    for (int c = threadIdx.x; c < kPassAlleles; c += kCompatThreads) col_sum[c] = 0;
+    __syncthreads();
+  }
   constexpr int32_t kHi999 = 0x3FEFF7CE, kLo999 = (int32_t)0xD916872B, kHi001 = 0x3F50624D, kLo001 = (int32_t)0xD2F1A9FC;
   const int tid = threadIdx.x, lane = tid & 63;
   const int wid = __builtin_amdgcn_readfirstlane(tid >> 6);
@@ -512,6 +547,10 @@
             }
           }
           *reinterpret_cast<uint32_t*>(miss8 + (int64_t)(a_base + al) * ldm + row0 + r0) = packed;
+          if (kSum) {
+            const uint32_t four = __builtin_amdgcn_sad_u8(packed, 0u, 0u);
+            if (four) atomicAdd(&col_sum[al], four);
+          }
         }
       }
     }
@@ -524,6 +563,10 @@
       }
     }
     __syncthreads();
+  }
+  if (kSum) {
+    for (int c = threadIdx.x; c < n_pass; c += kCompatThreads)
+      if (col_sum[c]) atomicAdd(&msum[a_base + c], col_sum[c]);
   }
 }
 
@@ -556,7 +599,8 @@
 int launch_compat(gk_ctx* ctx, gk_tab* tab, gk_dptr d_rows, int64_t n_rows, gk_dptr d_vflag, int vbeg, int vend,
                   gk_dptr d_mask, int words, int n_allele, double* out, uint8_t* miss, uint16_t* nvar, LutView view,
                   int keep_empty, uint8_t* miss8 = nullptr, int64_t ldm = 0, uint32_t* bound_flags = nullptr,
-                  uint16_t* lidx = nullptr, const int32_t* table_cols = nullptr, int n_table_cols = 0) {
+                  uint16_t* lidx = nullptr, const int32_t* table_cols = nullptr, int n_table_cols = 0,
+                  uint32_t* msum = nullptr) {
   const double empty_p = keep_empty ? 0.999 : 1.0;
   const int words_in = words;
   int32_t* d_cols = nullptr;
@@ -581,21 +625,28 @@
   }
   if (n_mask > 0 && d_cols)
     GK_KERNEL(transpose_gather_mask, dim3((unsigned)((n_mask + kThreads - 1) / kThreads)), dim3(kThreads), 0, ctx->stream,
-              gk_ptr<uint32_t>(d_mask), vend - vbeg, words_in, d_cols, n_table_cols, words, mask_t, bound_flags);
+              gk_ptr<uint32_t>(d_mask), vend - vbeg, words_in, d_cols, n_table_cols, words, mask_t, bound_flags, msum, n_allele);
   else if (n_mask > 0)
     GK_KERNEL(transpose_mask, dim3((unsigned)((n_mask + kThreads - 1) / kThreads)), dim3(kThreads), 0, ctx->stream,
-              gk_ptr<uint32_t>(d_mask), vend - vbeg, words, mask_t, bound_flags);
-  else if (bound_flags)
-    GK_HIP(hipMemsetAsync(bound_flags, 0, sizeof(uint32_t), ctx->stream));
+              gk_ptr<uint32_t>(d_mask), vend - vbeg, words, mask_t, bound_flags, msum, n_allele);
+  else {
+    if (bound_flags) GK_HIP(hipMemsetAsync(bound_flags, 0, sizeof(uint32_t), ctx->stream));
+    if (msum) GK_HIP(hipMemsetAsync(msum, 0, (size_t)n_allele * sizeof(uint32_t), ctx->stream));
+  }
   for (int a_base = 0; a_base < n_allele; a_base += 64 * kMaxSlots) {
     const int slots = std::min(kMaxSlots, (n_allele - a_base + 63) / 64);
 #define GK_COMPAT_GO(S, IDX)                                                                                        \
   GK_KERNEL((compat_kernel<kLog, S, !kLog, IDX>), grid, block, 0, ctx->stream, gk_ptr<int32_t>(d_rows), n_rows,     \
             tab->d_off, tab->d_ids, gk_ptr<uint8_t>(d_vflag), vbeg, vend, mask_t, words, n_allele, a_base, out,     \
-            miss, nvar, view, empty_p, miss8, ldm, bound_flags, lidx)
+            miss, nvar, view, empty_p, miss8, ldm, bound_flags, lidx, (uint32_t*)nullptr)
+#define GK_COMPAT_GO_SUM(S)                                                                                         \
+  GK_KERNEL((compat_kernel<kLog, S, !kLog, false, kLog>), grid, block, 0, ctx->stream, gk_ptr<int32_t>(d_rows),    \
+            n_rows, tab->d_off, tab->d_ids, gk_ptr<uint8_t>(d_vflag), vbeg, vend, mask_t, words, n_allele, a_base,  \
+            out, miss, nvar, view, empty_p, miss8, ldm, bound_flags, lidx, msum)
 #define GK_COMPAT_LAUNCH(S)                              \
   GK_PROF(ctx, "compat_kernel", {                        \
     if (kLog && lidx) GK_COMPAT_GO(S, (kLog && true));   \
+    else if (kLog && msum) GK_COMPAT_GO_SUM(S);          \
     else GK_COMPAT_GO(S, false);                         \
   })
     switch (slots) {
@@ -605,6 +656,7 @@
       default: GK_COMPAT_LAUNCH(4); break;
     }
 #undef GK_COMPAT_LAUNCH
+#undef GK_COMPAT_GO_SUM
 #undef GK_COMPAT_GO
   }
   gk_pool_free(ctx, mask_t);
@@ -819,11 +871,15 @@
   int64_t* n_out = nullptr;
   uint64_t* novel_key = nullptr;
 };
+struct ExonHint {
+  gk_dptr xflag = 0;
+  gk_dptr maybe_exon = 0;
+};
 }
 
 static int sample_prepare(gk_ctx* ctx, gk_tab* tab, int32_t multiple, gk_dptr d_vflag, gk_dptr d_cnt, gk_dptr d_rows,
                           int64_t* gene_off_out, const Survivors* surv, bool keep_vflag = false, int rounds = 1,
-                          gk_dptr d_cnt_full = 0);
+                          gk_dptr d_cnt_full = 0, ExonHint hint = ExonHint());
 
 int gk_sample_prepare(gk_ctx* ctx, gk_tab* tab, int32_t multiple, gk_dptr d_vflag, gk_dptr d_cnt, gk_dptr d_rows,
                       int64_t* gene_off_out) {
@@ -858,8 +914,35 @@
   return sample_prepare(ctx, tab, multiple, d_vflag, d_cnt, d_rows, gene_off_out, &s, true, 2, d_cnt_full);
 }
 
+int gk_sample_prepare_all_exon(gk_ctx* ctx, gk_tab* tab, int32_t multiple, gk_dptr d_vflag, gk_dptr d_cnt, gk_dptr d_rows,
+                               int64_t* gene_off_out, int64_t max_out, int32_t* ord_out, uint32_t* pos_out,
+                               uint32_t* neg_out, int64_t* n_out, uint64_t* novel_key_out, gk_dptr d_exon_flags,
+                               gk_dptr d_maybe_exon) {
+  GK_REQUIRE(ord_out && pos_out && neg_out && n_out && max_out >= 0, "null pointer");
+  GK_REQUIRE(d_exon_flags && d_maybe_exon, "null exon hint");
+  Survivors s;
+  s.max_out = max_out; s.ord = ord_out; s.pos = pos_out; s.neg = neg_out; s.n_out = n_out; s.novel_key = novel_key_out;
+  ExonHint hint;
+  hint.xflag = d_exon_flags; hint.maybe_exon = d_maybe_exon;
+  return sample_prepare(ctx, tab, multiple, d_vflag, d_cnt, d_rows, gene_off_out, &s, false, 1, 0, hint);
+}
+
+int gk_sample_prepare_exon_nowalk(gk_ctx* ctx, gk_tab* tab, int32_t multiple, gk_dptr d_vflag, gk_dptr d_cnt, gk_dptr d_rows,
+                                  int64_t* gene_off_out, int64_t max_out, int32_t* ord_out, uint32_t* pos_out,
+                                  uint32_t* neg_out, int64_t* n_out, gk_dptr d_cnt_full, gk_dptr d_maybe_exon) {
+  GK_REQUIRE(ord_out && pos_out && neg_out && n_out && max_out >= 0, "null pointer");
+  GK_REQUIRE(d_cnt_full && d_maybe_exon, "the full model's tallies and its exon hint are needed");
+  GK_REQUIRE(d_cnt_full != d_cnt, "the full model's tallies and the exon model's are two buffers");
+  Survivors s;
+  s.max_out = max_out; s.ord = ord_out; s.pos = pos_out; s.neg = neg_out; s.n_out = n_out; s.novel_key = nullptr;
+  ExonHint hint;
+  hint.maybe_exon = d_maybe_exon;
+  return sample_prepare(ctx, tab, multiple, d_vflag, d_cnt, d_rows, gene_off_out, &s, true, 2, d_cnt_full, hint);
+}
+
 static int sample_prepare(gk_ctx* ctx, gk_tab* tab, int32_t multiple, gk_dptr d_vflag, gk_dptr d_cnt, gk_dptr d_rows,
-                          int64_t* gene_off_out, const Survivors* surv, bool keep_vflag, int rounds, gk_dptr d_cnt_full) {
+                          int64_t* gene_off_out, const Survivors* surv, bool keep_vflag, int rounds, gk_dptr d_cnt_full,
+                          ExonHint hint) {
   gk_bind(ctx);
   GK_REQUIRE(ctx && tab && tab->idx && d_vflag && d_cnt && d_rows && gene_off_out, "null pointer");
   if (surv) *surv->n_out = 0;
@@ -869,6 +952,10 @@
   for (int g = 0; g <= n_gene; ++g) gene_off_out[g] = 0;
   if (!keep_vflag) GK_HIP(hipMemsetAsync(gk_ptr<void>(d_vflag), 0, (size_t)std::max<int64_t>(nv, 1), st));
   GK_HIP(hipMemsetAsync(gk_ptr<void>(d_cnt), 0, (size_t)std::max<int64_t>(2 * nv, 1) * sizeof(uint32_t), st));
+  const bool write_hint = hint.xflag != 0, nowalk = hint.maybe_exon != 0 && !write_hint;
+  GK_REQUIRE(!write_hint || (!keep_vflag && rounds == 1), "the exon hint is written by a walk whose drop flags are all zero");
+  if (write_hint && tab->n_valid > 0)
+    GK_HIP(hipMemsetAsync(gk_ptr<void>(hint.maybe_exon), 0, (size_t)tab->n_valid, st));
   auto novel_only = [&]() -> int {
     if (surv && surv->novel_key && tab->n_novel > 0)
       GK_HIP(gk_fetch(ctx, surv->novel_key, tab->d_novel_key, (size_t)tab->n_novel * sizeof(uint64_t)));
@@ -915,20 +1002,31 @@
   uint32_t* cnt = gk_ptr<uint32_t>(d_cnt);
   uint8_t* vflag = gk_ptr<uint8_t>(d_vflag);
   uint8_t *maybe = nullptr, *alive = nullptr;
-  GK_HIP(gk_pool_malloc(ctx, (void**)&maybe, (size_t)tab->n_valid));
+  const bool own_maybe = !nowalk && !write_hint;
+  if (own_maybe) GK_HIP(gk_pool_malloc(ctx, (void**)&maybe, (size_t)tab->n_valid));
   GK_HIP(gk_pool_malloc(ctx, (void**)&alive, (size_t)tab->n_valid));
-  GK_HIP(hipMemsetAsync(maybe, 0, (size_t)tab->n_valid, st));
+  if (own_maybe) GK_HIP(hipMemsetAsync(maybe, 0, (size_t)tab->n_valid, st));
   for (int round = 0; round < rounds; ++round) {
-    if (round) GK_HIP(hipMemsetAsync(cnt, 0, (size_t)(2 * nv) * sizeof(uint32_t), st));
-    if (round == 0 && rounds > 1 && d_cnt_full) {
+    const bool from_full = d_cnt_full && (nowalk || (round == 0 && rounds > 1));
+    if (round && !from_full) GK_HIP(hipMemsetAsync(cnt, 0, (size_t)(2 * nv) * sizeof(uint32_t), st));
+    if (from_full) {
       const uint32_t* full = gk_ptr<const uint32_t>(d_cnt_full);
       GK_PROF(ctx, "mask_tallies", GK_KERNEL(mask_tallies, dim3(nblk(nv)), dim3(kThreads), 0, st, full, full + nv, vflag, nv, cnt, cnt + nv));
     } else {
-      GK_PROF(ctx, "count_ids_genes",
-              GK_KERNEL(count_ids_genes, dim3((unsigned)n_wg), dim3(kThreads), (size_t)max_local * 8 + kThreads * sizeof(uint32_t), st, part.d_rows,
-                        (const int32_t*)d_tab, (const int64_t*)(d_tab + o_row0), (const int64_t*)(d_tab + o_row1),
-                        tab->idx->d_gene_vbeg, max_local, tab->d_off, tab->d_ids, vflag, cnt, cnt + nv,
-                        round == rounds - 1 ? maybe : (uint8_t*)nullptr));
+      const size_t lds = (size_t)max_local * 8 + kThreads * sizeof(uint32_t);
+      uint8_t* const last = round == rounds - 1 ? maybe : (uint8_t*)nullptr;
+      if (write_hint)
+        GK_PROF(ctx, "count_ids_genes",
+                GK_KERNEL(count_ids_genes<true>, dim3((unsigned)n_wg), dim3(kThreads), lds, st, part.d_rows,
+                          (const int32_t*)d_tab, (const int64_t*)(d_tab + o_row0), (const int64_t*)(d_tab + o_row1),
+                          tab->idx->d_gene_vbeg, max_local, tab->d_off, tab->d_ids, vflag, cnt, cnt + nv, last,
+                          gk_ptr<const uint8_t>(hint.xflag), gk_ptr<uint8_t>(hint.maybe_exon)));
+      else
+        GK_PROF(ctx, "count_ids_genes",
+                GK_KERNEL(count_ids_genes<false>, dim3((unsigned)n_wg), dim3(kThreads), lds, st, part.d_rows,
+                          (const int32_t*)d_tab, (const int64_t*)(d_tab + o_row0), (const int64_t*)(d_tab + o_row1),
+                          tab->idx->d_gene_vbeg, max_local, tab->d_off, tab->d_ids, vflag, cnt, cnt + nv, last,
+                          (const uint8_t*)nullptr, (uint8_t*)nullptr));
     }
     GK_PROF(ctx, "apply_correction", GK_KERNEL(apply_correction, dim3(nblk(nv)), dim3(kThreads), 0, st, cnt, cnt + nv, nv, vflag));
   }
@@ -936,13 +1034,15 @@
   GK_HIP(gk_pool_malloc(ctx, (void**)&flag, (size_t)n_rows * sizeof(uint32_t)));
   GK_HIP(gk_pool_malloc(ctx, (void**)&kept, (size_t)n_gene * sizeof(uint32_t)));
   GK_PROF(ctx, "flag_pairs", GK_KERNEL(flag_pairs, dim3(nblk(4 * (int64_t)tab->n_valid)), dim3(kThreads), 0, st, (int64_t)tab->n_valid,
-                                   tab->d_off, tab->d_ids, vflag, maybe, alive));
+                                   tab->d_off, tab->d_ids, vflag, own_maybe ? maybe : gk_ptr<const uint8_t>(hint.maybe_exon),
+                                   (uint8_t)(nowalk ? 2 : 0xFF), alive));
   GK_PROF(ctx, "gather_pair_flags", GK_KERNEL(gather_pair_flags, dim3(nblk(std::max<int64_t>(n_rows, n_gene))), dim3(kThreads), 0, st,
                                           part.d_rows, n_rows, alive, flag, kept, n_gene));
   GK_PROF(ctx, "count_flags_per_gene", GK_KERNEL(count_flags_per_gene, dim3((unsigned)n_gene, kFlagSlices), dim3(kThreads), 0, st, flag,
                                       (const int64_t*)(d_tab + o_goff), kept));
   GK_HIP(hipGetLastError());
-  std::vector<void*> temps{flag, kept, d_tab, alive, maybe};
+  std::vector<void*> temps{flag, kept, d_tab, alive};
+  if (maybe) temps.push_back(maybe);
   auto done = [&](int code) {
     for (void* t : temps) gk_pool_free(ctx, t);
     return code;
@@ -1058,6 +1158,35 @@
                              gk_ptr<uint8_t>(d_miss8), ldm, gk_ptr<uint32_t>(d_flags), nullptr, table_cols, n_table_cols);
 }
 
+int gk_compat_log_miss_sums(gk_ctx* ctx, gk_tab* tab, gk_dptr d_rows, int64_t n_rows, gk_dptr d_vflag, int32_t vbeg,
+                            int32_t vend, gk_dptr d_mask, int32_t words, int32_t n_allele, int32_t keep_empty, gk_lut* lut,
+                            const int32_t* table_cols, int32_t n_table_cols, gk_dptr d_log, gk_dptr d_miss8, int64_t ldm,
+                            gk_dptr d_flags, gk_dptr d_msum) {
+  gk_bind(ctx);
+  GK_REQUIRE(ctx && tab && lut, "null pointer");
+  GK_REQUIRE(words >= 1 && n_allele >= 0 && n_allele <= words * 32 && vend >= vbeg, "bad mask geometry");
+  GK_REQUIRE(d_msum, "null output");
+  if (table_cols) {
+    GK_REQUIRE(n_table_cols >= 1 && n_table_cols <= n_allele, "bad column list");
+    for (int c = 0; c < n_table_cols; ++c)
+      GK_REQUIRE(table_cols[c] >= 0 && table_cols[c] < n_allele && (c == 0 || table_cols[c] > table_cols[c - 1]),
+                 "table columns must be allele ordinals, ascending and unique");
+  } else {
+    n_table_cols = 0;
+  }
+  const int n_cols = table_cols ? n_table_cols : n_allele;
+  if (n_rows == 0 || n_cols == 0) {
+    if (n_cols) GK_HIP(hipMemsetAsync(gk_ptr<void>(d_msum), 0, (size_t)n_cols * sizeof(uint32_t), ctx->stream));
+    return GK_OK;
+  }
+  GK_REQUIRE(d_log && d_miss8 && d_flags, "null output");
+  GK_REQUIRE(ldm >= n_rows && ldm % 64 == 0, "mismatch table stride must be a multiple of 64 rows");
+  return launch_compat<true>(ctx, tab, d_rows, n_rows, d_vflag, vbeg, vend, d_mask, words, n_allele,
+                             gk_ptr<double>(d_log), nullptr, nullptr, gk_lut_view(lut), keep_empty,
+                             gk_ptr<uint8_t>(d_miss8), ldm, gk_ptr<uint32_t>(d_flags), nullptr, table_cols, n_table_cols,
+                             gk_ptr<uint32_t>(d_msum));
+}
+
 int gk_compat_patch(gk_ctx* ctx, gk_lut* lut, gk_dptr d_log, int64_t n_rows, int32_t n_allele, gk_dptr d_miss8, int64_t ldm,
                     gk_dptr d_flags) {
   gk_bind(ctx);
diff --git a/kir_graph_amd/engine.py b/kir_graph_amd/engine.py
--- a/kir_graph_amd/engine.py
+++ b/kir_graph_amd/engine.py
@@ -11,6 +11,7 @@
 from ._lib import Device, DeviceBuffer, DeviceSlice, TabInfo, check, lib
 from .index import GkIndex, KEY_POS_SHIFT, KEY_TYP_SHIFT, KEY_VAL_MASK
 from .msa2hisat import Variant
+from .utils import testHook
 
 TYPE_OF_RANK = {0: "insertion", 1: "single", 2: "deletion"}
 
@@ -52,6 +53,7 @@
     rows: DeviceBuffer
     off: np.ndarray
     surviving: Surviving
+    maybe_exon: DeviceBuffer | None = None
 
     def gene(self, g: int, vbeg: int, vend: int, dev: Device | None = None) -> PreparedGene:
         a, b = int(self.off[g]), int(self.off[g + 1])
@@ -150,13 +152,21 @@
     def close(self) -> None:
         if self.handle and not getattr(self, "_borrowed", False):
             for prep in (getattr(self, "_prepared", None) or {}).values():
-                for b in (prep.vflag, prep.cnt, prep.rows):
-                    b.free()
+                for b in (prep.vflag, prep.cnt, prep.rows, prep.maybe_exon):
+                    if b is not None:
+                        b.free()
             self._prepared = {}
             lib().gk_tab_destroy(self.handle)
         self.handle = None
 
-    def prepared(self, dev: Device, multiple: bool = False, exon: bool = False) -> PreparedSample | None:
+    def _exonFlags(self, nv: int) -> np.ndarray:
+        host = self.dindex.host
+        flags = np.full(nv, 3, dtype=np.uint8)
+        flags[:host.n_variant][host.in_exon.astype(bool)] = 0
+        return flags
+
+    def prepared(self, dev: Device, multiple: bool = False, exon: bool = False,
+                 exon_follows: bool = False) -> PreparedSample | None:
         if self.dindex is None or not self.info.d_pair_src:
             return None
         root = getattr(self, "_root", self)
@@ -169,9 +179,7 @@
                 host = self.dindex.host
                 nv = max(self.n_var_total, 1)
                 if exon:
-                    flags = np.full(nv, 3, dtype=np.uint8)
-                    flags[:host.n_variant][host.in_exon.astype(bool)] = 0
-                    vflag = dev.put(flags)
+                    vflag = dev.put(self._exonFlags(nv))
                 else:
                     vflag = dev.alloc(nv, np.uint8)
                 cnt = dev.alloc(2 * nv, np.uint32)
@@ -179,26 +187,42 @@
                 off = np.zeros(len(host.genes) + 1, dtype=np.int64)
                 o, p, q = (np.empty(nv, dtype=t) for t in (np.int32, np.uint32, np.uint32))
                 n_surv = C.c_int64()
+                maybe_exon = None
                 args = (dev.ctx, self.handle, int(multiple), vflag.ptr, cnt.ptr, rows.ptr, off.ctypes.data, nv,
                         o.ctypes.data, p.ctypes.data, q.ctypes.data, C.byref(n_surv))
                 if exon:
                     full = store.get(bool(multiple))
-                    if full is not None:
+                    walks = 2 if full is None else 0 if full.maybe_exon is not None else 1
+                    if full is not None and full.maybe_exon is not None:
+                        check(lib().gk_sample_prepare_exon_nowalk(*args, full.cnt.ptr, full.maybe_exon.ptr))
+                    elif full is not None:
                         check(lib().gk_sample_prepare_exon_from(*args, full.cnt.ptr))
                     else:
                         check(lib().gk_sample_prepare_exon(*args))
                 else:
+                    walks = 1
                     want_novel = self._novel_keys is None and self.n_novel > 0
                     novel_keys = np.empty(self.n_novel, dtype=np.uint64) if want_novel else None
-                    check(lib().gk_sample_prepare_all(*args, novel_keys.ctypes.data if want_novel else None))
+                    keys_ptr = novel_keys.ctypes.data if want_novel else None
+                    if exon_follows and testHook("exon_walk") is None:
+                        xflag = dev.put(self._exonFlags(nv))
+                        maybe_exon = dev.alloc(max(self.n_valid, 1), np.uint8)
+                        check(lib().gk_sample_prepare_all_exon(*args, keys_ptr, xflag.ptr, maybe_exon.ptr))
+                        xflag.free()
+                    else:
+                        check(lib().gk_sample_prepare_all(*args, keys_ptr))
                     if want_novel:
                         self._novel_keys = root._novel_keys = novel_keys
+                if dev.call_log is not None:
+                    dev.call_log.append(("count_ids_genes", self.n_valid, self.n_ids, walks, 1))
+                    dev.call_log.append(("flag_pairs", self.n_valid, 1.0))
                 o, p, q = o[:n_surv.value], p[:n_surv.value], q[:n_surv.value]
                 gene_of = np.searchsorted(host.gene_vbeg, o, side="right") - 1
                 if not exon and len(o) and int(o[-1]) >= host.n_variant:
                     is_novel = o >= host.n_variant
                     gene_of[is_novel] = (self.novelKeys()[o[is_novel] - host.n_variant] >> np.uint64(56)).astype(gene_of.dtype)
-                prep = store[key] = PreparedSample(vflag, cnt, rows, off, _groupByGene(gene_of, o, p, q, len(host.genes)))
+                prep = store[key] = PreparedSample(vflag, cnt, rows, off, _groupByGene(gene_of, o, p, q, len(host.genes)),
+                                                   maybe_exon)
         return prep
 
     @staticmethod
diff --git a/kir_graph_amd/kir_typing.py b/kir_graph_amd/kir_typing.py
--- a/kir_graph_amd/kir_typing.py
+++ b/kir_graph_amd/kir_typing.py
@@ -227,7 +227,7 @@
         full_tables = testHook("full_tables") is not None
         tab, logs = self._context()
         udev = tab.dev.urgent()
-        prep_f = tab.prepared(udev, self._multiple)
+        prep_f = tab.prepared(udev, self._multiple, exon_follows=True)
         if prep_f is None:
             return super().typing(gene_cn, min_reads_num)
         prep_e = tab.prepared(udev, self._multiple, exon=True)
diff --git a/kir_graph_amd/roofmodel.py b/kir_graph_amd/roofmodel.py
--- a/kir_graph_amd/roofmodel.py
+++ b/kir_graph_amd/roofmodel.py
@@ -49,6 +49,14 @@
 def tabLaunch(n_pairs: int, n_valid: int, n_ids: int, record_bytes: float | None = None) -> tuple[float, float]:
     read = 256.0 * n_pairs if record_bytes is None else float(record_bytes)
     return read + 4.0 * n_ids + 22.0 * n_valid, 0.0
+
+
+def prepareLaunch(n_rows: int, n_ids: float, walks: int, notes: int = 1) -> tuple[float, float]:
+    return walks * (20.0 * n_rows + 4.0 * n_ids) + (float(notes) * n_rows if walks else 0.0), 0.0
+
+
+def flagPairsLaunch(n_pairs: int, marked: float = 1.0) -> tuple[float, float]:
+    return 2.0 * n_pairs + 32.0 * marked * n_pairs, 0.0
 
 
 def setsumLaunch(n_rows: int, n_sets: int, c: int, n_distinct: int) -> tuple[float, float]:
@@ -86,6 +94,10 @@
             b, o = compatLaunch(*c[1:5])[0], 0.0
         elif kernel == "tab_count":
             b, o = tabLaunch(*c[1:5])
+        elif kernel == "count_ids_genes":
+            b, o = prepareLaunch(*c[1:5])
+        elif kernel == "flag_pairs":
+            b, o = flagPairsLaunch(*c[1:3])
         elif kernel in ("fraction_chunks", "setsum_leaves"):
             b, o = setsumLaunch(*c[1:5])
         else:
```

New measurement: 540.4 million, median of 3. No clear change (+0.4%).
